# Tcadart/pyLatticeDSO

Measured on AMD Instinct MI355X. Metric: beams/s assembly+PCG-solve, higher is better.
Workload: dtype f64

## Files before the change

pylatticedso_amd/csrc/pl_api.hip:

```cpp
#include "pl_solver.h"
#include "pl_condense.h"
#include "pl_multi.h"


namespace {
template <typename WT>
int debug_spd_solve_t(int device, int32_t n, const double *A, const double *b, double *x, double *quad) {
  if (n <= 0 || !A || !b || !x) return fail(PL_ERR_ARG, "pl_debug_spd_solve: bad argument");
  int ndev = 0;
  if (hipGetDeviceCount(&ndev) != hipSuccess || ndev <= 0) return fail(PL_ERR_NODEVICE, "no HIP device visible");
  PL_HIP(hipSetDevice(device));
  const int np = (n + pl::kNB - 1) / pl::kNB * pl::kNB;
  std::vector<double> Ap((size_t)np * np, 0.0), bp(np, 0.0);
  for (int i = 0; i < np; ++i) {
    if (i < n) {
      std::memcpy(&Ap[(size_t)i * np], A + (size_t)i * n, n * sizeof(double));
      bp[i] = b[i];
    } else {
      Ap[(size_t)i * np + i] = 1.0;
    }
  }
  DevBuf<double> dA, dL, dD, db, dt, dy, dq;
  DevBuf<WT> dW, dWt;
  DevBuf<int> dinfo;
// ... 18 lines not shown
  PL_HIP(hipGetLastError());
  PL_HIP(hipDeviceSynchronize());
  int info[2];
  PL_HIP(hipMemcpy(info, dinfo.p, sizeof(info), hipMemcpyDeviceToHost));
  if (info[0] != 0) return fail(PL_ERR_ARG, "pl_debug_spd_solve: matrix is not positive definite");
  std::vector<double> y(np), q(pl::kSlots);
  PL_HIP(hipMemcpy(y.data(), dy.p, np * sizeof(double), hipMemcpyDeviceToHost));
  PL_HIP(hipMemcpy(q.data(), dq.p, pl::kSlots * sizeof(double), hipMemcpyDeviceToHost));
  std::memcpy(x, y.data(), n * sizeof(double));
  if (quad) {
    *quad = 0.0;
    for (double v : q) *quad += v;
  }
  return PL_OK;
}

}

extern "C" {

const char *pl_last_error(void) { return g_err.c_str(); }
#ifndef PL_KP_HASH
#define PL_KP_HASH "unknown"
#endif
const char *pl_version(void) { return "pylattice_hip 0.2 (gfx950) kp=" PL_KP_HASH; }

uint32_t pl_opts_size(void) { return (uint32_t)sizeof(pl_opts_t); }
uint32_t pl_stats_size(void) { return (uint32_t)sizeof(pl_stats_t); }
uint32_t pl_abi_version(void) { return PL_ABI_VERSION; }

int pl_default_opts(pl_opts_t *o, uint32_t struct_size) {
  if (!o) return fail(PL_ERR_ARG, "pl_default_opts: null argument");
  if (struct_size != sizeof(pl_opts_t))
    return fail(PL_ERR_ARG, "pl_default_opts: the caller's pl_opts_t has " + std::to_string(struct_size) +
                                " bytes, this library's " + std::to_string(sizeof(pl_opts_t)) +
                                " (ABI version " + std::to_string(PL_ABI_VERSION) + "): rebuild the binding against include/pylattice_hip.h");
  std::memset(o, 0, sizeof(*o));
  o->struct_size = (uint32_t)sizeof(pl_opts_t);
  o->abi_version = PL_ABI_VERSION;
  o->young = 1013.0;
  o->poisson = 0.3;
  o->kappa = 0.9;
  o->pen_coef = 1.5;
  o->device = 0;
  o->spmv_kernel = 0;
  o->precond = 1;
  o->reorder = 1;
  o->check_every = 0;
  return PL_OK;
}

namespace {
int check_opts_abi(const pl_opts_t *o, const char *who) {
  if (o->struct_size != sizeof(pl_opts_t) || o->abi_version != PL_ABI_VERSION)
    return fail(PL_ERR_ARG, std::string(who) + ": pl_opts_t was not initialised by pl_default_opts of this library (struct_size " +
                                std::to_string(o->struct_size) + " / abi " + std::to_string(o->abi_version) + ", expected " +
                                std::to_string(sizeof(pl_opts_t)) + " / " + std::to_string(PL_ABI_VERSION) + ")");
  return PL_OK;
}
inline bool multi_rank_handle(const pl_opts_t *o) { return o->grid_nodes > 0; }
inline int coarse_modes_of(const pl_opts_t *o, int64_t N = -1) {
  const bool tile12 = o->precond == 3 && o->tile_modes != 6;
  if (!tile12 || o->coarse_modes == 6) return 6;
  if (multi_rank_handle(o)) N = o->grid_nodes;
  return (o->coarse_modes == 12 || N < 0 || N >= 250000) ? 12 : 6;
}
inline int coarse_budget(const pl_opts_t *o, int64_t N) {
  const bool multi_rank = o->grid_nodes > 0;
  if (o->coarse_max_dofs > 0) return o->coarse_max_dofs;
  if (multi_rank) return (coarse_modes_of(o, N) == 12 && o->grid_nodes >= 2000000) ? 6144 : 3072;
  if (coarse_modes_of(o, N) == 12) return N >= 2000000 ? 6144 : (N >= 1000000 ? 3072 : (N >= 250000 ? 1536 : 768));
  return N >= 1000000 ? 3072 : 2100;
}
}

int pl_create(const pl_mesh_t *m, const pl_opts_t *o, pl_handle *out) {
  if (!m || !o || !out) return fail(PL_ERR_ARG, "pl_create: null argument");
  if (int rc_abi = check_opts_abi(o, "pl_create")) return rc_abi;
  StageTimer stage("pl_create");
  if (m->n_nodes <= 0 || m->n_beams <= 0) return fail(PL_ERR_ARG, "pl_create: empty mesh");
  if (m->n_nodes >= (1LL << 31) - 64 || m->n_beams >= (1LL << 31) - 64)
    return fail(PL_ERR_ARG, "pl_create: more than 2^31 nodes/struts per handle");
  if (!m->node_xyz || !m->beam_conn || !m->beam_radius || !m->seg_len || !m->seg_nsub)
    return fail(PL_ERR_ARG, "pl_create: null mesh array");
  int ndev = 0;
  if (hipGetDeviceCount(&ndev) != hipSuccess || ndev <= 0)
    return fail(PL_ERR_NODEVICE, "pl_create: no HIP device visible (libpylattice_hip has no CPU fallback)");
  if (o->device < 0 || o->device >= ndev) return fail(PL_ERR_ARG, "pl_create: bad device ordinal");
  if (o->precond == 5 && 6 * m->n_nodes > PL_DDM_DENSE_MAX)
    return fail(PL_ERR_ARG, "pl_create: precond = 5 (dense factorisation) serves at most PL_DDM_DENSE_MAX dofs");
  const int64_t N = m->n_nodes, B = m->n_beams;
  {
    std::atomic<int64_t> bad_ends{-1}, bad_radius{-1}, bad_len{-1}, bad_seg{-1};
    pl::parallel_for(B, [&](int64_t b0, int64_t b1, unsigned) {
      for (int64_t b = b0; b < b1; ++b) {
        const int32_t a = m->beam_conn[2 * b], d = m->beam_conn[2 * b + 1];
        if (a < 0 || d < 0 || a >= N || d >= N || a == d) bad_ends = b;
        if (!(m->beam_radius[b] > 0.0)) bad_radius = b;
        const double L = m->seg_len[3 * b] + m->seg_len[3 * b + 1] + m->seg_len[3 * b + 2];
        if (!(L > 0.0)) bad_len = b;
        for (int k = 0; k < 3; ++k)
          if (m->seg_len[3 * b + k] < 0.0 || (m->seg_len[3 * b + k] > 0.0 && m->seg_nsub[3 * b + k] < 1)) bad_seg = b;
      }
    });
    if (bad_ends >= 0)
      return fail(PL_ERR_ARG, "pl_create: strut " + std::to_string(bad_ends.load()) + " has invalid end nodes");
    if (bad_radius >= 0) return fail(PL_ERR_ARG, "pl_create: non-positive radius");
    if (bad_len >= 0) return fail(PL_ERR_ARG, "pl_create: strut with zero length");
    if (bad_seg >= 0) return fail(PL_ERR_ARG, "pl_create: bad segment data on strut " + std::to_string(bad_seg.load()));
  }
  stage.mark("validate");
  PL_HIP(hipSetDevice(o->device));
  pl_context *c = new pl_context();
  c->opt = *o;
  c->N = N;
  c->B = B;
  c->mat = {o->young, o->young / (2.0 * (1.0 + o->poisson)), o->kappa, o->pen_coef};
  c->lpn = o->lanes_per_node > 0 ? o->lanes_per_node : pl::kDefaultLPN;
  if (c->lpn != 1 && c->lpn != 2 && c->lpn != 4 && c->lpn != 8 && c->lpn != 16) {
    delete c;
    return fail(PL_ERR_ARG, "pl_create: lanes_per_node must be 0 (default), 1, 2, 4, 8 or 16");
  }
  auto bail = [&](int rc) {
    delete c;
    return rc;
  };
#define PL_TRY(expr)              \
  do {                            \
    int _rc = (expr);             \
    if (_rc) return bail(_rc);    \
  } while (0)
#define PL_HIPC(expr)                                                                  \
  do {                                                                                 \
    hipError_t _e = (expr);                                                            \
    if (_e != hipSuccess)                                                              \
      return bail(fail(PL_ERR_HIP, std::string(#expr) + ": " + hipGetErrorString(_e))); \
  } while (0)
  {
    int prio_low = 0, prio_high = 0;
    PL_HIPC(hipDeviceGetStreamPriorityRange(&prio_low, &prio_high));
    PL_HIPC(hipStreamCreateWithPriority(&c->stream, hipStreamNonBlocking, prio_high));
    PL_HIPC(hipStreamCreateWithPriority(&c->side, hipStreamNonBlocking, prio_low));
  }
  PL_HIPC(hipEventCreate(&c->ev0));
  PL_HIPC(hipEventCreate(&c->ev1));
  PL_HIPC(hipEventCreateWithFlags(&c->ev_fork, hipEventDisableTiming));
  PL_HIPC(hipEventCreateWithFlags(&c->ev_join, hipEventDisableTiming));
  PL_HIPC(hipEventCreateWithFlags(&c->ev_chol, hipEventDisableTiming));
  PL_HIPC(hipEventCreateWithFlags(&c->ev_t0, hipEventDisableTiming));
  PL_HIPC(hipEventCreateWithFlags(&c->ev_t1, hipEventDisableTiming));
  PL_HIPC(hipEventCreateWithFlags(&c->ev_p0, hipEventDisableTiming));
  PL_HIPC(hipEventCreateWithFlags(&c->ev_p1, hipEventDisableTiming));
  PL_HIPC(hipEventCreateWithFlags(&c->ev_fill1, hipEventDisableTiming));
  PL_HIPC(hipStreamCreateWithFlags(&c->side2, hipStreamNonBlocking));
  {
    const char *e = std::getenv("PL_BSR_CUMASK");
    const int k = e ? std::atoi(e) : 4;
    hipDeviceProp_t prop;
    const bool tuned_layout = hipGetDeviceProperties(&prop, o->device) == hipSuccess && prop.multiProcessorCount == 256;
    if (k > 0 && k < 8 && tuned_layout) {
      uint32_t mask[8];
      for (int w = 0; w < 8; ++w) {
        mask[w] = 0u;
        for (int b = 0; b < 32; ++b) {
          const int i = 32 * w + b;
          if ((i / 8 + i) % 8 >= k) mask[w] |= 1u << b;
        }
      }
      if (hipExtStreamCreateWithCUMask(&c->side_cu, 8, mask) != hipSuccess) {
        (void)hipGetLastError();
        c->side_cu = nullptr;
      }
    }
  }

  const double global_grid[7] = {o->grid_lo[0], o->grid_lo[1], o->grid_lo[2], o->grid_hi[0], o->grid_hi[1],
                                 o->grid_hi[2], (double)o->grid_nodes};
  c->perm.resize(N);
  std::iota(c->perm.begin(), c->perm.end(), 0);
  std::vector<int32_t> tile_start, tile_of;
  std::vector<int64_t> tile_brick;
  pl::BrickGrid grid;
  if (o->reorder == 1) {
    pl::spatial_order(m->node_xyz, N, c->perm, tile_start,
                      (double)(o->tile_nodes > 0 ? std::min(o->tile_nodes, pl::kTileMaxNodes) : 256), tile_brick,
                      grid, o->grid_nodes > 0 ? global_grid : nullptr,
                      (o->precond >= 2 && o->precond <= 4) ? coarse_budget(o, N) * 6 / coarse_modes_of(o, N) : 0);
    c->reordered = true;
    {
      std::vector<uint64_t> kind((size_t)N, 0);
      pl::parallel_for(B, [&](int64_t b0, int64_t b1, unsigned) {
        for (int64_t b = b0; b < b1; ++b) {
          const int32_t u = m->beam_conn[2 * b], v = m->beam_conn[2 * b + 1];
          uint64_t d = 0;
          for (int k = 0; k < 3; ++k) {
            const int64_t q = (int64_t)std::llround((m->node_xyz[3 * (size_t)v + k] - m->node_xyz[3 * (size_t)u + k]) * 4096.0);
            d = d * 0x9E3779B97F4A7C15ull + (uint64_t)(q + (1 << 20));
          }
          auto mix = [](uint64_t h) { h ^= h >> 33; h *= 0xFF51AFD7ED558CCDull; h ^= h >> 33; return h; };
          __atomic_fetch_add(&kind[u], mix(d), __ATOMIC_RELAXED);
          __atomic_fetch_add(&kind[v], mix(~d), __ATOMIC_RELAXED);
        }
      }, 1 << 16);
      const int64_t T = (int64_t)tile_start.size() - 1;
      pl::parallel_for(T, [&](int64_t t0, int64_t t1, unsigned) {
        for (int64_t t = t0; t < t1; ++t)
          std::stable_sort(c->perm.begin() + tile_start[t], c->perm.begin() + tile_start[t + 1],
                           [&](int32_t l, int32_t r) { return kind[l] < kind[r]; });
      }, 16);
    }
  } else {
    pl::chunk_tiles(N, tile_start);
  }
  stage.mark("spatial order");
  c->iperm.resize(N);
  pl::parallel_for(N, [&](int64_t i0, int64_t i1, unsigned) {
    for (int64_t i = i0; i < i1; ++i) c->iperm[c->perm[i]] = (int32_t)i;
  }, 1 << 16);
  if (o->condense >= 0 && o->precond >= 2 && o->precond <= 4 && o->precision != 2 && o->reorder == 1) {
    std::vector<int64_t> aptr((size_t)N + 1, 0);
    pl::parallel_for(2 * B, [&](int64_t k0, int64_t k1, unsigned) {
      for (int64_t k = k0; k < k1; ++k)
        __atomic_fetch_add(&aptr[c->iperm[m->beam_conn[k]] + 1], (int64_t)1, __ATOMIC_RELAXED);
    }, 1 << 16);
    for (int64_t i = 0; i < N; ++i) aptr[i + 1] += aptr[i];
    std::vector<int32_t> adj((size_t)2 * B);
    {
      std::vector<int64_t> fill(aptr.begin(), aptr.end() - 1);
      pl::parallel_for(B, [&](int64_t b0, int64_t b1, unsigned) {
        for (int64_t b = b0; b < b1; ++b) {
          const int32_t u = c->iperm[m->beam_conn[2 * b]], v = c->iperm[m->beam_conn[2 * b + 1]];
          adj[__atomic_fetch_add(&fill[u], (int64_t)1, __ATOMIC_RELAXED)] = v;
          adj[__atomic_fetch_add(&fill[v], (int64_t)1, __ATOMIC_RELAXED)] = u;
        }
      }, 1 << 16);
    }
    double lo[3] = {1e300, 1e300, 1e300}, hi[3] = {-1e300, -1e300, -1e300};
    for (int64_t i = 0; i < N; ++i)
      for (int k = 0; k < 3; ++k) {
        lo[k] = std::min(lo[k], m->node_xyz[3 * i + k]);
        hi[k] = std::max(hi[k], m->node_xyz[3 * i + k]);
      }
    std::vector<uint8_t> state((size_t)N, 0);
    for (int pass = 0; pass < 2; ++pass)
      for (int64_t i = 0; i < N; ++i) {
        if (state[i] || aptr[i + 1] - aptr[i] < 3) continue;
        const double *q3 = m->node_xyz + 3 * (size_t)c->perm[i];
        const bool on_box = q3[0] <= lo[0] || q3[0] >= hi[0] || q3[1] <= lo[1] || q3[1] >= hi[1] || q3[2] <= lo[2] ||
                            q3[2] >= hi[2];
        if (on_box != (pass == 1)) continue;
        state[i] = 1;
        for (int64_t q = aptr[i]; q < aptr[i + 1]; ++q)
          if (!state[adj[q]]) state[adj[q]] = 2;
      }
    int64_t n_cand = 0;
    for (int64_t i = 0; i < N; ++i) n_cand += state[i] == 1;
    const bool use = o->condense > 0 || (double)n_cand >= 0.45 * (double)N;
    const int64_t T = use ? (int64_t)tile_start.size() - 1 : 0;
    std::vector<int32_t> np(c->perm.size());
    if (use) c->h_cand.assign((size_t)N, 0);
    for (int64_t t = 0; t < T; ++t) {
      int64_t w = tile_start[t];
      for (int pass = 0; pass < 2; ++pass)
        for (int64_t i = tile_start[t]; i < tile_start[t + 1]; ++i)
          if ((state[i] == 1) == (pass == 1)) {
            c->h_cand[w] = (uint8_t)pass;
            np[w++] = c->perm[i];
          }
    }
    if (use) {
      c->perm.swap(np);
      for (int64_t i = 0; i < N; ++i) c->iperm[c->perm[i]] = (int32_t)i;
    }
  }

  stage.mark("candidates");
  std::vector<double> xyz((size_t)N * 3);
  pl::parallel_for(N, [&](int64_t i0, int64_t i1, unsigned) {
    for (int64_t i = i0; i < i1; ++i)
      std::memcpy(&xyz[3 * i], m->node_xyz + 3 * (size_t)c->perm[i], 3 * sizeof(double));
  });
  std::vector<int32_t> conn((size_t)B * 2);
  {
    std::vector<int32_t> conn0((size_t)B * 2);
    pl::parallel_for(2 * B, [&](int64_t k0, int64_t k1, unsigned) {
      for (int64_t k = k0; k < k1; ++k) conn0[k] = c->iperm[m->beam_conn[k]];
    });
    pl::tile_strut_order(conn0, N, B, tile_start, tile_of, c->bperm, xyz.data());
    pl::parallel_for(B, [&](int64_t b0, int64_t b1, unsigned) {
      for (int64_t b = b0; b < b1; ++b) {
        conn[2 * b] = conn0[2 * (size_t)c->bperm[b]];
        conn[2 * b + 1] = conn0[2 * (size_t)c->bperm[b] + 1];
      }
    });
  }
  stage.mark("strut order");
  std::vector<double> radius(B), seg_len((size_t)B * 3);
  std::vector<int32_t> seg_nsub((size_t)B * 3);
  pl::parallel_for(B, [&](int64_t b0, int64_t b1, unsigned) {
    for (int64_t b = b0; b < b1; ++b) {
      const size_t ob = (size_t)c->bperm[b];
      radius[b] = m->beam_radius[ob];
      for (int k = 0; k < 3; ++k) {
        seg_len[3 * b + k] = m->seg_len[3 * ob + k];
        seg_nsub[3 * b + k] = m->seg_nsub[3 * ob + k];
      }
    }
// ... 400 lines not shown
    if (cell_S[c] < 0 || cell_S[c] >= n_S) return fail(PL_ERR_ARG, "pl_ddm_set_preconditioner: matrix id out of range");
  const int m = 6 * h->ddm_nb;
  std::vector<double> Pt((size_t)n_S * m * m);
  for (int s = 0; s < n_S; ++s)
    for (int i = 0; i < m; ++i)
      for (int j = 0; j < m; ++j) Pt[((size_t)s * m + j) * m + i] = S[((size_t)s * m + i) * m + j];
  PL_HIP(h->ddm_Pt.alloc(Pt.size()));
  PL_HIP(h->ddm_cell_P.alloc(h->ddm_cells));
  PL_HIP(hipMemcpy(h->ddm_Pt.p, Pt.data(), Pt.size() * sizeof(double), hipMemcpyHostToDevice));
  PL_HIP(hipMemcpy(h->ddm_cell_P.p, cell_S, h->ddm_cells * sizeof(int32_t), hipMemcpyHostToDevice));
  h->ddm_have_P = true;
  return PL_OK;
}

static int ensure_bsr_buffers(pl_context *h) {
  if (h->bsr_vals.p) return PL_OK;
  PL_HIP(h->bsr_rowptr.alloc(h->N + 1));
  PL_HIP(h->bsr_col.alloc(h->nblk));
  PL_HIP(h->bsr_vals.alloc((size_t)h->nblk * 36));
  PL_HIP(hipMemcpy(h->bsr_rowptr.p, h->h_rowptr.data(), (h->N + 1) * sizeof(int64_t), hipMemcpyHostToDevice));
  PL_HIP(hipMemcpy(h->bsr_col.p, h->h_col.data(), h->nblk * sizeof(int32_t), hipMemcpyHostToDevice));
  return PL_OK;
}

static int ddm_factor_preconditioner(pl_context *h) {
  const int64_t n6 = h->N * 6;
  const int np = (int)((n6 + pl::kNB - 1) / pl::kNB * pl::kNB);
  if (h->dd_n != np) {
    const size_t nn = (size_t)np * np;
    PL_HIP(h->dd_A.alloc(nn));
    PL_HIP(h->dd_Lf.alloc(nn));
    PL_HIP(h->dd_W.alloc(nn));
    PL_HIP(h->dd_Wt.alloc(nn));
    PL_HIP(h->dd_Dinv.alloc((size_t)np * pl::kNB));
    PL_HIP(h->dd_tv.alloc(np));
    PL_HIP(h->dd_info.alloc(2));
    PL_HIP(hipMemsetAsync(h->dd_W.p, 0, nn * sizeof(double), h->stream));
    PL_HIP(hipMemsetAsync(h->dd_Wt.p, 0, nn * sizeof(double), h->stream));
    h->dd_n = np;
  }
  h->dd_ready = false;
  PL_HIP(hipMemsetAsync(h->dd_A.p, 0, (size_t)np * np * sizeof(double), h->stream));
  PL_HIP(hipMemsetAsync(h->dd_info.p, 0, 2 * sizeof(int), h->stream));
  const int m = 6 * h->ddm_nb;
  const int64_t ne = h->ddm_cells * m * m;
  const uint8_t *fx = h->have_bc ? h->fixed.p : (const uint8_t *)nullptr;
  hipLaunchKernelGGL(pl::k_ddm_dense_assemble, dim3(grid_for(ne)), dim3(pl::kBlock), 0, h->stream, h->ddm_cells,
                     h->ddm_nb, h->ddm_cell_nodes.p, h->ddm_have_P ? h->ddm_cell_P.p : h->ddm_cell_S.p,
                     h->ddm_have_P ? h->ddm_Pt.p : h->ddm_St.p, fx, np, h->dd_A.p);
  hipLaunchKernelGGL(pl::k_ddm_dense_unit, dim3((np + 255) / 256), dim3(256), 0, h->stream, n6, np, fx, h->dd_A.p);
  pl::dense_factor_inverse(h->dd_A.p, h->dd_Lf.p, h->dd_W.p, h->dd_Wt.p, h->dd_Dinv.p, np, np, h->dd_info.p,
                           h->dd_bw, h->stream);
  PL_HIP(hipGetLastError());
  int info[2] = {0, 0};
  PL_HIP(hipMemcpyAsync(info, h->dd_info.p, sizeof(info), hipMemcpyDeviceToHost, h->stream));
  PL_HIP(hipStreamSynchronize(h->stream));
  h->dd_ready = (info[0] == 0);
  return PL_OK;
}

static int fem_factor_dense(pl_context *h) {
  const int64_t n6 = h->N * 6;
  const int np = (int)((n6 + pl::kNB - 1) / pl::kNB * pl::kNB);
  if (h->dd_n != np) {
    const size_t nn = (size_t)np * np;
    PL_HIP(h->dd_A.alloc(nn));
    PL_HIP(h->dd_Lf.alloc(nn));
    PL_HIP(h->dd_W.alloc(nn));
    PL_HIP(h->dd_Wt.alloc(nn));
    PL_HIP(h->dd_Dinv.alloc((size_t)np * pl::kNB));
    PL_HIP(h->dd_tv.alloc(np));
    PL_HIP(h->dd_info.alloc(2));
    PL_HIP(hipMemsetAsync(h->dd_W.p, 0, nn * sizeof(double), h->stream));
    PL_HIP(hipMemsetAsync(h->dd_Wt.p, 0, nn * sizeof(double), h->stream));
    h->dd_n = np;
    int64_t band = 0;
    for (int64_t i = 0; i < h->N; ++i)
      for (int64_t q = h->h_rowptr[i]; q < h->h_rowptr[i + 1]; ++q) band = std::max<int64_t>(band, std::llabs((long long)(h->h_col[q] - i)));
    h->dd_bw = (int)((6 * (band + 1) + pl::kNB - 1) / pl::kNB + 1);
  }
  h->dd_ready = false;
  int rc = ensure_bsr_buffers(h);
  if (rc) return rc;
  PL_HIP(hipMemsetAsync(h->dd_A.p, 0, (size_t)np * np * sizeof(double), h->stream));
  PL_HIP(hipMemsetAsync(h->dd_info.p, 0, 2 * sizeof(int), h->stream));
  rc = launch_bsr_fill(h, 1, h->stream);
  if (rc) return rc;
  h->have_bsr = false;
  hipLaunchKernelGGL(pl::k_bsr_to_dense, dim3(grid_for(h->nblk * 36)), dim3(pl::kBlock), 0, h->stream, h->N, h->nblk,
                     h->bsr_rowptr.p, h->bsr_col.p, (const double *)h->bsr_vals.p, np, h->dd_A.p);
  hipLaunchKernelGGL(pl::k_ddm_dense_unit, dim3((np + 255) / 256), dim3(256), 0, h->stream, n6, np, (const uint8_t *)nullptr,
                     h->dd_A.p);
  pl::dense_factor_inverse(h->dd_A.p, h->dd_Lf.p, h->dd_W.p, h->dd_Wt.p, h->dd_Dinv.p, np, np, h->dd_info.p, h->dd_bw,
                           h->stream);
  PL_HIP(hipGetLastError());
  int info[2] = {0, 0};
  PL_HIP(hipMemcpyAsync(info, h->dd_info.p, sizeof(info), hipMemcpyDeviceToHost, h->stream));
  PL_HIP(hipStreamSynchronize(h->stream));
  h->dd_ready = (info[0] == 0);
  if (h->dd_ready) PL_HIP(hipMemsetAsync(h->dinv.p, 0, n6 * sizeof(double), h->stream));
  return PL_OK;
}

void pl_destroy(pl_handle h) {
  if (!h) return;
  (void)hipSetDevice(h->opt.device);
  (void)hipStreamSynchronize(h->stream);
  if (h->comm_stream) (void)hipStreamSynchronize(h->comm_stream);
  pl::dist_destroy(h->dist);
  if (h->pal_host_flags != h->pal_fallback_flags) (void)hipHostFree(h->pal_host_flags);
  if (h->cls_host_flag) (void)hipHostFree(h->cls_host_flag);
  delete h;
}

int pl_set_bc(pl_handle h, const uint8_t *fixed, const double *ubar, const double *f) {
  if (!valid(h) || !fixed) return fail(PL_ERR_ARG, "pl_set_bc: null argument");
  PL_HIP(hipSetDevice(h->opt.device));
  const int64_t N = h->N;
  const size_t n6 = (size_t)N * 6;
  std::vector<uint8_t> fx(n6), bits(N);
  double *st = nullptr;
  if (int rcs = staging(h, &st)) return rcs;
  pl::parallel_for(N, [&](int64_t i0, int64_t i1, unsigned) {
    for (int64_t i = i0; i < i1; ++i) {
      const size_t src = 6 * (size_t)h->perm[i];
      uint8_t b = 0;
      for (int k = 0; k < 6; ++k) {
        const uint8_t v = fixed[src + k] ? 1 : 0;
        fx[6 * i + k] = v;
        b |= (uint8_t)(v << k);
        st[6 * i + k] = (ubar && v) ? ubar[src + k] : 0.0;
      }
      bits[i] = b;
    }
  }, 1 << 15);
  PL_HIP(hipMemcpyAsync(h->ubar.p, st, n6 * sizeof(double), hipMemcpyHostToDevice, h->stream));
  PL_HIP(hipMemcpyAsync(h->fixed.p, fx.data(), n6, hipMemcpyHostToDevice, h->stream));
  PL_HIP(hipMemcpyAsync(h->fixedbits.p, bits.data(), N, hipMemcpyHostToDevice, h->stream));
  PL_HIP(hipStreamSynchronize(h->stream));
  pl::parallel_for(N, [&](int64_t i0, int64_t i1, unsigned) {
    for (int64_t i = i0; i < i1; ++i) {
      const size_t src = 6 * (size_t)h->perm[i];
      for (int k = 0; k < 6; ++k) st[6 * i + k] = f ? f[src + k] : 0.0;
    }
  }, 1 << 15);
  PL_HIP(hipMemcpyAsync(h->f.p, st, n6 * sizeof(double), hipMemcpyHostToDevice, h->stream));
  PL_HIP(hipStreamSynchronize(h->stream));
  const bool same_mask = h->have_bc && !h->dist.active && h->h_fixedbits == bits;
  h->h_fixedbits = bits;
  if (same_mask) return PL_OK;
  h->have_bc = true;
  h->coarse.n_fix = -1;
  h->coarseL.n_fix = -1;
  {
    int rcs = select_condensed(h, bits);
    if (rcs) return rcs;
  }
  if (h->assembled && h->opkind == 1) {
    if (h->opt.precond >= 2 && h->opt.precond <= 4) {
      h->assembled = false;
      h->dd_ready = false;
      h->dd_blocks = false;
      h->dd2_ready = false;
    } else {
      pl::launch_invert_diag(h->N * 6, h->diag.p, h->fixed.p, h->dinv.p, h->stream);
      PL_HIP(hipStreamSynchronize(h->stream));
    }
  } else if (h->assembled) {
    int rc = launch_diag(h, h->stream);
    if (rc) return rc;
    rc = finish_diag_dist(h);
    if (rc) return rc;
    rc = launch_local_mask(h);
    if (rc) return rc;
    rc = launch_tile_blocks(h, h->stream);
    if (rc) return rc;
    rc = build_coarse(h);
    if (rc) return rc;
    rc = launch_dinv32(h);
    if (rc) return rc;
    rc = agree_condensed(h);
    if (rc) return rc;
    rc = launch_condensed_blocks(h, h->stream);
    if (rc) return rc;
    PL_HIP(hipStreamSynchronize(h->stream));
    {
      const bool keep = h->pal_ready;
      finish_condensed_classes(h);
      (void)keep;
    }
    if (h->bsr_with_bc) h->have_bsr = false;
    if (h->opt.precond == 5 && !h->dist.active) {
      rc = fem_factor_dense(h);
      if (rc) return rc;
    }
  }
  return PL_OK;
}

int pl_set_periodic(pl_handle h, const int32_t *master) {
  if (!valid(h)) return fail(PL_ERR_ARG, "pl_set_periodic: null handle");
  if (h->opkind != 0) return fail(PL_ERR_STATE, "pl_set_periodic: not available on a DDM handle");
  h->n_per_groups = 0;
  if (!master) return PL_OK;
  if (h->opt.precond != 1 || h->dist.active)
    return fail(PL_ERR_STATE, "pl_set_periodic: periodic constraints are served by the Jacobi PCG of a single-GPU handle (opts.precond = 1)");
  PL_HIP(hipSetDevice(h->opt.device));
  const int64_t N = h->N;
  std::vector<int32_t> inv((size_t)N);
  for (int64_t i = 0; i < N; ++i) inv[(size_t)h->perm[i]] = (int32_t)i;
  std::vector<int32_t> cnt((size_t)N, 0);
  for (int64_t i = 0; i < N; ++i) {
    const int32_t m = master[i];
    if (m < 0 || m >= N || master[m] != m) return fail(PL_ERR_ARG, "pl_set_periodic: master[i] must name a node that is its own master");
    cnt[(size_t)m]++;
  }
  std::vector<int32_t> ptr(1, 0), nodes, start((size_t)N, -1);
  for (int64_t m = 0; m < N; ++m)
    if (cnt[(size_t)m] >= 2) {
      start[(size_t)m] = (int32_t)ptr.size() - 1;
      ptr.push_back(ptr.back() + cnt[(size_t)m]);
    }
  nodes.resize((size_t)ptr.back());
  std::vector<int32_t> fill(ptr.begin(), ptr.end() - 1);
  for (int64_t i = 0; i < N; ++i) {
    const int32_t g = start[(size_t)master[i]];
    if (g >= 0) nodes[(size_t)fill[(size_t)g]++] = inv[(size_t)i];
  }
  const int64_t ng = (int64_t)ptr.size() - 1;
  if (ng == 0) return PL_OK;
  PL_HIP(h->per_ptr.alloc(ptr.size()));
  PL_HIP(h->per_nodes.alloc(nodes.size()));
  PL_HIP(hipMemcpy(h->per_ptr.p, ptr.data(), ptr.size() * sizeof(int32_t), hipMemcpyHostToDevice));
  PL_HIP(hipMemcpy(h->per_nodes.p, nodes.data(), nodes.size() * sizeof(int32_t), hipMemcpyHostToDevice));
  h->n_per_groups = ng;
  return PL_OK;
}

int pl_update_radii(pl_handle h, const double *beam_radius) {
  if (!valid(h) || !beam_radius) return fail(PL_ERR_ARG, "pl_update_radii: null argument");
  if (h->opkind != 0) return fail(PL_ERR_STATE, "pl_update_radii: not available on a DDM handle");
  for (int64_t b = 0; b < h->B; ++b)
    if (!(beam_radius[b] > 0.0)) return fail(PL_ERR_ARG, "pl_update_radii: non-positive radius");
  PL_HIP(hipSetDevice(h->opt.device));
  double *stg = nullptr;
  int rc = stagingB(h, &stg);
  if (rc) return rc;
  pl::parallel_for(h->B, [&](int64_t b0, int64_t b1, unsigned) {
    for (int64_t b = b0; b < b1; ++b) stg[b] = beam_radius[h->bperm[b]];
  }, 1 << 16);
  PL_HIP(hipMemcpyAsync(h->radius.p, stg, h->B * sizeof(double), hipMemcpyHostToDevice, h->stream));
  PL_HIP(hipStreamSynchronize(h->stream));
  h->assembled = false;
  h->have_bsr = false;
  return PL_OK;
}

int pl_set_multiplicity(pl_handle h, const double *beam_mult) {
  if (!valid(h)) return fail(PL_ERR_ARG, "pl_set_multiplicity: null handle");
  if (h->opkind != 0) return fail(PL_ERR_STATE, "pl_set_multiplicity: not available on a DDM handle");
  PL_HIP(hipSetDevice(h->opt.device));
  if (!beam_mult) {
    h->mult.release();
  } else {
    for (int64_t b = 0; b < h->B; ++b)
      if (!(beam_mult[b] > 0.0)) return fail(PL_ERR_ARG, "pl_set_multiplicity: non-positive multiplicity");
    std::vector<double> m(h->B);
    for (int64_t b = 0; b < h->B; ++b) m[b] = beam_mult[h->bperm[b]];
    if (!h->mult.p) PL_HIP(h->mult.alloc(h->B));
    PL_HIP(hipMemcpy(h->mult.p, m.data(), h->B * sizeof(double), hipMemcpyHostToDevice));
  }
  h->assembled = false;
  h->have_bsr = false;
  return PL_OK;
}

int pl_update_segments(pl_handle h, const double *seg_len, const int32_t *seg_nsub) {
  if (!valid(h) || !seg_len || !seg_nsub) return fail(PL_ERR_ARG, "pl_update_segments: null argument");
  PL_HIP(hipSetDevice(h->opt.device));
  std::vector<double> sl((size_t)h->B * 3);
  std::vector<int32_t> sn((size_t)h->B * 3);
  for (int64_t b = 0; b < h->B; ++b)
    for (int k = 0; k < 3; ++k) {
      sl[3 * b + k] = seg_len[3 * (size_t)h->bperm[b] + k];
      sn[3 * b + k] = seg_nsub[3 * (size_t)h->bperm[b] + k];
    }
  PL_HIP(hipMemcpy(h->seg_len.p, sl.data(), 3 * h->B * sizeof(double), hipMemcpyHostToDevice));
  PL_HIP(hipMemcpy(h->seg_nsub.p, sn.data(), 3 * h->B * sizeof(int32_t), hipMemcpyHostToDevice));
  h->assembled = false;
  h->have_bsr = false;
  return PL_OK;
}

int pl_assemble(pl_handle h) {
  if (!valid(h)) return fail(PL_ERR_ARG, "pl_assemble: null handle");
  PL_HIP(hipSetDevice(h->opt.device));
  if (h->opkind == 1) {
    if (h->assembled && (h->opt.precond == 0 || (h->opt.precond == 1 && !h->dd_ready && !h->dd_blocks) || h->dd_ready || h->dd_blocks)) {
      h->ms_assembly = 0.0;
      return PL_OK;
    }
    h->dd_ready = false;
    h->dd_blocks = false;
    h->dd2_ready = false;
    if (h->opt.precond == 4 && !h->dd2_plan)
      return fail(PL_ERR_STATE, "pl_assemble: precond = 4 on a DDM handle needs the node positions (pl_ddm_set_geometry)");
    if (h->opt.precond == 3 || h->opt.precond == 4) {
      PL_HIP(hipEventRecord(h->ev0, h->stream));
      if (!h->dd_B.p) PL_HIP(h->dd_B.alloc((size_t)h->N * 36));
      PL_HIP(hipMemsetAsync(h->dd_B.p, 0, (size_t)h->N * 36 * sizeof(double), h->stream));
      const int64_t ne = (int64_t)h->ddm_cells * h->ddm_nb * 36;
      hipLaunchKernelGGL(pl::k_ddm_node_blocks, dim3(grid_for(ne)), dim3(pl::kBlock), 0, h->stream, h->ddm_cells, h->ddm_nb,
                         h->ddm_cell_nodes.p, h->ddm_have_P ? h->ddm_cell_P.p : h->ddm_cell_S.p,
                         h->ddm_have_P ? h->ddm_Pt.p : h->ddm_St.p, h->dd_B.p);
      hipLaunchKernelGGL(pl::k_ddm_node_blocks_invert, dim3(grid_for(h->N)), dim3(pl::kBlock), 0, h->stream, h->N,
                         h->have_bc ? (const uint8_t *)h->fixed.p : (const uint8_t *)nullptr, h->dd_B.p);
      PL_HIP(hipMemsetAsync(h->dinv.p, 0, h->N * 6 * sizeof(double), h->stream));
      int info2[2] = {0, 0};
      if (h->opt.precond == 4) {
        pl::Coarse &cs = h->dd2;
        const int n = cs.ncp, m = 6 * h->ddm_nb;
        PL_HIP(hipMemsetAsync(cs.Ac, 0, (size_t)n * n * sizeof(double), h->stream));
        PL_HIP(hipMemsetAsync(cs.info, 0, 2 * sizeof(int), h->stream));
        hipLaunchKernelGGL(pl::k_ddm_coarse_cells, dim3((unsigned)h->ddm_cells), dim3(pl::kWave),
                           (size_t)2 * m * pl::kDdmModes * sizeof(double), h->stream, h->ddm_cells, h->ddm_nb,
                           h->ddm_cell_nodes.p, h->ddm_have_P ? h->ddm_cell_P.p : h->ddm_cell_S.p,
                           h->ddm_have_P ? h->ddm_Pt.p : h->ddm_St.p, h->dd2_agg.p, h->dd2_cen.p, h->dd2_xyz.p,
                           h->have_bc ? (const uint8_t *)h->fixed.p : (const uint8_t *)nullptr, n, cs.Ac);
        hipLaunchKernelGGL(pl::k_coarse_regularize, dim3((n + 255) / 256), dim3(256), 0, h->stream, n, cs.Ac);
        pl::TrtriPhases ph;
        ph.rows = 3;
        ph.stream = h->side2;
        ph.ev_go = h->ev_t0;
        ph.ev_done = h->ev_t1;
        pl::coarse_factor(cs, n, h->stream, nullptr, (unsigned *)nullptr, ph);
        cs.ainv_ready = false;
        if (cs.Ainv) {
          const long tiles = (long)(n / 32) * (n / 32 + 1) / 2;
          if (cs.w16)
            hipLaunchKernelGGL(pl::k_dense_explicit_inverse<pl::bf16_t>, dim3((unsigned)((tiles + 3) / 4)), dim3(256), 0,
                               h->stream, n, reinterpret_cast<const pl::bf16_t *>(cs.W), n, cs.Ainv);
          else
            hipLaunchKernelGGL(pl::k_dense_explicit_inverse<float>, dim3((unsigned)((tiles + 3) / 4)), dim3(256), 0, h->stream,
                               n, (const float *)cs.W, n, cs.Ainv);
          cs.ainv_ready = true;
        }
        PL_HIP(hipMemcpyAsync(info2, cs.info, sizeof(info2), hipMemcpyDeviceToHost, h->stream));
      }
      PL_HIP(hipEventRecord(h->ev1, h->stream));
      PL_HIP(hipEventSynchronize(h->ev1));
      PL_HIP(hipGetLastError());
      float ms = 0.f;
      PL_HIP(hipEventElapsedTime(&ms, h->ev0, h->ev1));
      h->ms_assembly = ms;
      h->dd2_ready = h->opt.precond == 4 && info2[0] == 0;
      h->dd_blocks = true;
      h->assembled = true;
      return PL_OK;
    }
    if (h->opt.precond == 2) {
      PL_HIP(hipEventRecord(h->ev0, h->stream));
      int rcp = ddm_factor_preconditioner(h);
      if (rcp) return rcp;
      if (h->dd_ready) {
        PL_HIP(hipMemsetAsync(h->dinv.p, 0, h->N * 6 * sizeof(double), h->stream));
        PL_HIP(hipEventRecord(h->ev1, h->stream));
        PL_HIP(hipEventSynchronize(h->ev1));
        float ms = 0.f;
        PL_HIP(hipEventElapsedTime(&ms, h->ev0, h->ev1));
        h->ms_assembly = ms;
        h->assembled = true;
        return PL_OK;
      }
    }
    if (h->opt.precond >= 1) {
      PL_HIP(hipMemsetAsync(h->diag.p, 0, h->N * 6 * sizeof(double), h->stream));
      const int64_t m = (int64_t)h->ddm_cells * h->ddm_nb * 6;
      hipLaunchKernelGGL(pl::k_ddm_diag, dim3(grid_for(m)), dim3(pl::kBlock), 0, h->stream, h->ddm_cells, h->ddm_nb,
                         h->ddm_cell_nodes.p, h->ddm_cell_S.p, h->ddm_St.p, h->diag.p);
    } else {
      pl::launch_fill(h->N * 6, 1.0, h->diag.p, h->stream);
    }
    pl::launch_invert_diag(h->N * 6, h->diag.p, h->have_bc ? h->fixed.p : nullptr, h->dinv.p, h->stream);
    PL_HIP(hipStreamSynchronize(h->stream));
    h->ms_assembly = 0.0;
    h->assembled = true;
    return PL_OK;
  }
  int rc = agree_condensed(h);
  if (rc) return rc;
  PL_HIP(hipEventRecord(h->ev0, h->stream));
  rc = launch_records(h);
  if (rc) return rc;
  rc = launch_local_mask(h);
  if (rc) return rc;
  PL_HIP(hipEventRecord(h->ev_fork, h->stream));
  PL_HIP(hipStreamWaitEvent(h->side, h->ev_fork, 0));
  rc = launch_palette(h, h->side);
  if (rc) return rc;
  rc = launch_diag(h, h->dist.active ? h->stream : h->side);
  if (rc) return rc;
  rc = finish_diag_dist(h);
  if (rc) return rc;
  rc = launch_tile_blocks(h, h->side);
  if (rc) return rc;
  rc = launch_condensed_blocks(h, h->side);
  if (rc) return rc;
  const bool refresh_bsr = h->want_bsr && (!h->bsr_with_bc || h->have_bc);
  int rc_fill = PL_OK;
  bool fill_queued = false;
  int64_t split = 0;
  if (refresh_bsr && h->side_cu && h->coarse.enabled && h->have_bc) {
    static const double kChainLinkMs = [] { const char *e = std::getenv("PL_CHAIN_LINK_MS"); return e ? std::atof(e) : 0.04; }();
    static const double kFillBlocksPerMs = [] { const char *e = std::getenv("PL_FILL_BLOCKS_PER_MS"); return e ? std::atof(e) : 8.5e6; }();
    const double chain_ms = kChainLinkMs * std::max(0, h->coarse.ncp / pl::kNB - 1);
    const double fit = chain_ms * kFillBlocksPerMs / std::max<double>(1.0, (double)h->nblk);
    split = fit >= 1.0 ? h->n_slices : (int64_t)(fit * (double)h->n_slices);
    if (split < h->n_slices / 16) split = 0;
  }
  bool part1_queued = false;
  auto queue_fill = [&](int phase) {
    if (!refresh_bsr || fill_queued) return;
    if (phase == 0) {
      if (split <= 0 || part1_queued) return;
      part1_queued = true;
      if (hipEventRecord(h->ev_chol, h->stream) != hipSuccess || hipStreamWaitEvent(h->side_cu, h->ev_chol, 0) != hipSuccess ||
          hipStreamWaitEvent(h->side_cu, h->ev_join, 0) != hipSuccess) {
        rc_fill = fail(PL_ERR_HIP, "pl_assemble: could not order the BSR fill beside the factorisation");
        return;
      }
      rc_fill = launch_bsr_fill(h, h->bsr_with_bc, h->side_cu, 0, split);
      if (hipEventRecord(h->ev_fill1, h->side_cu) != hipSuccess) rc_fill = fail(PL_ERR_HIP, "pl_assemble: event record failed");
      return;
    }
    fill_queued = true;
    if (hipEventRecord(h->ev_chol, h->stream) != hipSuccess || hipStreamWaitEvent(h->side, h->ev_chol, 0) != hipSuccess) {
      rc_fill = fail(PL_ERR_HIP, "pl_assemble: could not order the BSR fill behind the factorisation");
      return;
    }
    if (!rc_fill) rc_fill = launch_bsr_fill(h, h->bsr_with_bc, h->side, part1_queued ? split : 0, -1);
    if (part1_queued && hipStreamWaitEvent(h->side, h->ev_fill1, 0) != hipSuccess)
      rc_fill = fail(PL_ERR_HIP, "pl_assemble: event wait failed");
    if (hipEventRecord(h->ev_join, h->side) != hipSuccess) rc_fill = fail(PL_ERR_HIP, "pl_assemble: event record failed");
  };
  PL_HIP(hipEventRecord(h->ev_join, h->side));
  h->dd_ready = false;
  if (h->opt.precond == 5 && h->have_bc && !h->dist.active) {
    PL_HIP(hipStreamWaitEvent(h->stream, h->ev_join, 0));
    rc = fem_factor_dense(h);
    if (rc) return rc;
  }
  rc = build_coarse(h, h->coarse.enabled && h->have_bc ? std::function<void(int)>(queue_fill) : std::function<void(int)>());
  if (rc) return rc;
  queue_fill(1);
  if (rc_fill) return rc_fill;
  PL_HIP(hipStreamWaitEvent(h->stream, h->ev_join, 0));
  rc = launch_dinv32(h);
  if (rc) return rc;
  PL_HIP(hipEventRecord(h->ev1, h->stream));
  PL_HIP(hipStreamSynchronize(h->stream));
  finish_palette(h);
  finish_condensed_classes(h);
  for (pl::Coarse *cs : {&h->coarse, &h->coarseL})
    if (cs->ready && cs->Ac) {
      PL_HIP(hipMemsetAsync(cs->Ac, 0, (size_t)cs->ncp * cs->ncp * sizeof(double), h->stream));
      cs->ac_clean = true;
    }
  float ms = 0.f;
  PL_HIP(hipEventElapsedTime(&ms, h->ev0, h->ev1));
  h->ms_assembly = ms;
  h->assembled = true;
  h->have_bsr = refresh_bsr;
  return PL_OK;
}

int pl_assemble_bsr(pl_handle h, int with_bc, int64_t *n_block_rows, int64_t *n_blocks) {
  if (!valid(h)) return fail(PL_ERR_ARG, "pl_assemble_bsr: null handle");
  if (h->opkind != 0) return fail(PL_ERR_STATE, "pl_assemble_bsr: not available on a DDM handle");
  if (!h->assembled) return fail(PL_ERR_STATE, "pl_assemble_bsr: call pl_assemble first");
  if (with_bc && !h->have_bc) return fail(PL_ERR_STATE, "pl_assemble_bsr: with_bc needs pl_set_bc");
  PL_HIP(hipSetDevice(h->opt.device));
  if (int rcb = ensure_bsr_buffers(h)) return rcb;
  const bool fresh = h->have_bsr && h->want_bsr && h->bsr_with_bc == (with_bc ? 1 : 0);
  h->want_bsr = true;
  h->bsr_with_bc = with_bc ? 1 : 0;
  if (fresh) {
    if (n_block_rows) *n_block_rows = h->N;
    if (n_blocks) *n_blocks = h->nblk;
    return PL_OK;
  }
  PL_HIP(hipEventRecord(h->ev0, h->stream));
  int rc = launch_bsr_fill(h, with_bc, h->stream);
  if (rc) return rc;
  PL_HIP(hipEventRecord(h->ev1, h->stream));
  PL_HIP(hipStreamSynchronize(h->stream));
  float ms = 0.f;
  PL_HIP(hipEventElapsedTime(&ms, h->ev0, h->ev1));
  h->ms_assembly += ms;
  h->have_bsr = true;
  if (n_block_rows) *n_block_rows = h->N;
  if (n_blocks) *n_blocks = h->nblk;
  return PL_OK;
}

int pl_get_bsr(pl_handle h, int64_t *rowptr, int32_t *colidx, double *vals) {
  if (!valid(h)) return fail(PL_ERR_ARG, "pl_get_bsr: null handle");
  if (!h->have_bsr) return fail(PL_ERR_STATE, "pl_get_bsr: call pl_assemble_bsr first");
  PL_HIP(hipSetDevice(h->opt.device));
  std::vector<double> v((size_t)h->nblk * 36);
  PL_HIP(hipMemcpy(v.data(), h->bsr_vals.p, v.size() * sizeof(double), hipMemcpyDeviceToHost));
  if (!h->reordered) {
    if (rowptr) std::memcpy(rowptr, h->h_rowptr.data(), (h->N + 1) * sizeof(int64_t));
    if (colidx) std::memcpy(colidx, h->h_col.data(), h->nblk * sizeof(int32_t));
    if (vals) std::memcpy(vals, v.data(), v.size() * sizeof(double));
    return PL_OK;
  }
  std::vector<int64_t> rp(h->N + 1, 0);
  for (int64_t ci = 0; ci < h->N; ++ci) {
    const int64_t di = h->iperm[ci];
    rp[ci + 1] = rp[ci] + (h->h_rowptr[di + 1] - h->h_rowptr[di]);
  }
  if (rowptr) std::memcpy(rowptr, rp.data(), (h->N + 1) * sizeof(int64_t));
  std::vector<std::pair<int32_t, int64_t>> row;
  for (int64_t ci = 0; ci < h->N; ++ci) {
    const int64_t di = h->iperm[ci];
    row.clear();
    for (int64_t p = h->h_rowptr[di]; p < h->h_rowptr[di + 1]; ++p) row.push_back({h->perm[h->h_col[p]], p});
    std::stable_sort(row.begin(), row.end(), [](auto &l, auto &r) { return l.first < r.first; });
    for (size_t k = 0; k < row.size(); ++k) {
      if (colidx) colidx[rp[ci] + k] = row[k].first;
      if (vals) std::memcpy(vals + 36 * (rp[ci] + k), &v[36 * row[k].second], 36 * sizeof(double));
    }
  }
  return PL_OK;
}

static int spmv_common(pl_handle h, const double *x, double *y, bool masked, const char *who) {
  if (!valid(h) || !x || !y) return fail(PL_ERR_ARG, std::string(who) + ": null argument");
  if (!h->assembled) return fail(PL_ERR_STATE, std::string(who) + ": call pl_assemble first");
  if (masked && !h->have_bc) return fail(PL_ERR_STATE, std::string(who) + ": call pl_set_bc first");
  PL_HIP(hipSetDevice(h->opt.device));
  std::vector<double> stage;
  int rc = upload6(h, x, h->tmp.p, stage);
  if (rc) return rc;
  if (masked) {
    hipLaunchKernelGGL(pl::k_mask_dot, dim3(grid_stream(h->N * 6)), dim3(pl::kBlock), 0, h->stream, h->N * 6,
                       h->fixed.p, h->tmp.p, h->tmp.p, (double *)nullptr);
  }
  rc = launch_spmv(h, h->tmp.p, h->tmp2.p, masked, nullptr);
  if (rc) return rc;
  return download6(h, h->tmp2.p, y);
}

int pl_spmv(pl_handle h, const double *x, double *y) { return spmv_common(h, x, y, false, "pl_spmv"); }
int pl_spmv_free(pl_handle h, const double *x, double *y) { return spmv_common(h, x, y, true, "pl_spmv_free"); }

int pl_spmv_bsr(pl_handle h, const double *x, double *y) {
  if (!valid(h) || !x || !y) return fail(PL_ERR_ARG, "pl_spmv_bsr: null argument");
  if (!h->have_bsr) return fail(PL_ERR_STATE, "pl_spmv_bsr: call pl_assemble_bsr first");
  PL_HIP(hipSetDevice(h->opt.device));
  std::vector<double> stage;
  int rc = upload6(h, x, h->tmp.p, stage);
  if (rc) return rc;
  hipLaunchKernelGGL(pl::k_bsr_spmv, dim3(grid_for(h->N)), dim3(pl::kBlock), 0, h->stream, h->N, h->bsr_rowptr.p,
                     h->bsr_col.p, h->bsr_vals.p, h->tmp.p, h->tmp2.p);
  PL_HIP(hipGetLastError());
  return download6(h, h->tmp2.p, y);
}

int pl_solve(pl_handle h, double rtol, int32_t max_iter, double *u, pl_stats_t *stats) {
  if (!valid(h)) return fail(PL_ERR_ARG, "pl_solve: null handle");
  if (!h->assembled) return fail(PL_ERR_STATE, "pl_solve: call pl_assemble first");
  if (!h->have_bc) return fail(PL_ERR_STATE, "pl_solve: call pl_set_bc first");
  if (!(rtol > 0.0) || max_iter <= 0) return fail(PL_ERR_ARG, "pl_solve: rtol and max_iter must be positive");
  if (stats && stats->struct_size != sizeof(pl_stats_t))
    return fail(PL_ERR_ARG, "pl_solve: stats->struct_size is " + std::to_string(stats->struct_size) + ", this library's pl_stats_t has " +
                                std::to_string(sizeof(pl_stats_t)) + " bytes (set it to sizeof(pl_stats_t) before the call)");
  PL_HIP(hipSetDevice(h->opt.device));
  const int64_t n6 = h->N * 6;
  pl_stats_t st{};
  st.struct_size = (uint32_t)sizeof(pl_stats_t);
  PL_HIP(hipEventRecord(h->ev0, h->stream));
  int rc = launch_spmv(h, h->ubar.p, h->tmp.p, false, nullptr);
  if (rc) return rc;
  if (h->n_per_groups > 0 && (h->coarse.ready || ref_cg(h) || h->dist.active))
    return fail(PL_ERR_STATE, "pl_solve: periodic constraints (pl_set_periodic) need the plain Jacobi PCG");
  const bool mp = mp_applies(h);
  solver_plan(h);
  const bool cg1 = !mp && cg1_applies(h);
  st.cg_form_used = cg1 ? 1.0 : 0.0;
  if (cg1) rc = pcg_solve_cg1(h, h->f.p, h->tmp.p, rtol, max_iter, &st);
  else if (mp && h->opt.precision == 1) rc = pcg_solve_mp_t<float>(h, h->f.p, h->tmp.p, rtol, max_iter, &st);
  else if (mp) rc = pcg_solve_mp_t<double>(h, h->f.p, h->tmp.p, rtol, max_iter, &st);
  else rc = pcg_solve(h, h->f.p, h->tmp.p, rtol, max_iter, &st);
  if (rc) return rc;
  st.precision_used = mp ? (double)h->opt.precision : 0.0;
  st.kp_form = (double)kp_form_of(h);
  st.comm_world = h->dist.active ? (double)h->dist.comm_count : 0.0;
  st.comm_rank = h->dist.active ? (double)h->dist.comm_user_rank : 0.0;
  st.condensed_nodes = h->cond_use ? (double)h->n_cond : 0.0;
  if (st.converged) st.info = 0.0;
  else if (st.info != 2.0) st.info = 1.0;
  if (!h->usol.p) PL_HIP(h->usol.alloc((size_t)n6));
  h->usol_valid = false;
  hipLaunchKernelGGL(pl::k_compose_solution, dim3(grid_stream(n6)), dim3(pl::kBlock), 0, h->stream, n6, h->fixed.p,
                     h->ubar.p, h->x.p, h->usol.p);
  PL_HIP(hipEventRecord(h->ev1, h->stream));
  PL_HIP(hipStreamSynchronize(h->stream));
  float ms = 0.f;
  PL_HIP(hipEventElapsedTime(&ms, h->ev0, h->ev1));
  st.ms_solve = ms;
  st.ms_assembly = h->ms_assembly;
  st.precond_used = h->opkind == 1 ? (h->dd_ready ? 2 : h->dd2_ready ? 4 : h->dd_blocks ? 3 : h->opt.precond >= 1 ? 1 : 0)
                                   : (h->coarse.ready ? h->opt.precond : (h->dd_ready ? 5 : 1));
// ... 452 lines not shown
  a.nb = nb;
  a.ni = ni;
  a.conn = dconn.p;
  a.end_slot = dslot.p;
  a.node_slot = dnslot.p;
  a.xyz = dxyz.p;
  a.radius = drad.p;
  a.seg_len = dlen.p;
  a.seg_nsub = dnsub.p;
  a.m = {o->young, o->young / (2.0 * (1.0 + o->poisson)), o->kappa, o->pen_coef};
  a.u_b = dub.p;
  a.lam_b = lam_b ? dlb.p : nullptr;
  a.u_full = u_full ? duf.p : nullptr;
  a.lam_full = lam_full ? dlf.p : nullptr;
  a.sens = sens ? dsens.p : nullptr;
  a.info = dinfo.p;
  if (lds > 64 * 1024)
    PL_HIP(hipFuncSetAttribute(reinterpret_cast<const void *>(&pl::k_cells_recover),
                               hipFuncAttributeMaxDynamicSharedMemorySize, (int)lds));
  KernelEventTimer kernel_time("pl_cells_recover", stage.on);
  hipLaunchKernelGGL(pl::k_cells_recover, dim3((unsigned)n_inst), dim3((unsigned)block), lds, nullptr, a);
  kernel_time.stop();
  PL_HIP(hipGetLastError());
  PL_HIP(hipDeviceSynchronize());
  kernel_time.report();
  stage.mark("kernel");
  if (u_full) PL_HIP(hipMemcpy(u_full, duf.p, duf.n * sizeof(double), hipMemcpyDeviceToHost));
  if (lam_full) PL_HIP(hipMemcpy(lam_full, dlf.p, dlf.n * sizeof(double), hipMemcpyDeviceToHost));
  if (sens) PL_HIP(hipMemcpy(sens, dsens.p, dsens.n * sizeof(double), hipMemcpyDeviceToHost));
  PL_HIP(hipMemcpy(info, dinfo.p, ninst * sizeof(int32_t), hipMemcpyDeviceToHost));
  stage.mark("download");
  return PL_OK;
}

int pl_get_records(pl_handle h, double *rec) {
  if (!valid(h) || !rec) return fail(PL_ERR_ARG, "pl_get_records: null argument");
  if (!h->assembled) return fail(PL_ERR_STATE, "pl_get_records: call pl_assemble first");
  PL_HIP(hipSetDevice(h->opt.device));
  std::vector<pl::Record> tmp(h->B);
  PL_HIP(hipMemcpy(tmp.data(), h->rec.p, h->B * sizeof(pl::Record), hipMemcpyDeviceToHost));
  for (int64_t b = 0; b < h->B; ++b) std::memcpy(rec + 8 * (size_t)h->bperm[b], &tmp[b], sizeof(pl::Record));
  return PL_OK;
}

int pl_algorithmic_bytes(pl_handle h, double *out3) {
  if (!valid(h) || !out3) return fail(PL_ERR_ARG, "pl_algorithmic_bytes: null argument");
  const double w = 8.0, B = (double)h->B, N = (double)h->N;
  const bool mp = h->assembled && mp_applies(h);
  const double wv = mp ? 4.0 : 8.0;
  const double wx = (mp && h->opt.precision == 1) ? 4.0 : 8.0;
  out3[0] = B * (8.0 + 8.0 * w) + N * 6.0 * wv * 2.0;
  out3[1] = out3[0] + 10.0 * (6.0 * N * wx);
  out3[2] = B * (8.0 + 8.0 * w) + (N + 2.0 * B) * (36.0 * w + 4.0);
  return PL_OK;
}

int pl_forget_history(pl_handle h) {
  if (!valid(h)) return fail(PL_ERR_ARG, "pl_forget_history: null handle");
  h->last_iterations = 0;
  h->xprev_valid = false;
  h->xprev2_valid = false;
  h->xprev3_valid = false;
  h->gh_count = 0;
  return PL_OK;
}

int pl_time_kernel(pl_handle h, int which, int reps, double *avg_ms) {
  if (!valid(h) || !avg_ms || reps <= 0) return fail(PL_ERR_ARG, "pl_time_kernel: bad argument");
  if (h->opkind != 0 && which != 0 && which != 3 && which != 10 && which != 11) return fail(PL_ERR_STATE, "pl_time_kernel: DDM handles time K*p / PCG only");
  if (!h->assembled) return fail(PL_ERR_STATE, "pl_time_kernel: call pl_assemble first");
  if ((which == 0 || which == 3 || which == 10 || which == 11) && !h->have_bc) return fail(PL_ERR_STATE, "pl_time_kernel: call pl_set_bc first");
  if ((which == 2 || which == 4) && !h->have_bsr) return fail(PL_ERR_STATE, "pl_time_kernel: needs pl_assemble_bsr");
  PL_HIP(hipSetDevice(h->opt.device));
  const int64_t n6 = h->N * 6;
  int rc = ensure_hist(h, reps + 1);
  if (rc) return rc;
  solver_plan(h);
  h->stop_use = false;
  if (h->small_use && (which == 3 || which == 11)) {
    rc = small_prepare(h);
    if (rc) return rc;
  }
  PL_HIP(hipMemcpyAsync(h->p.p, h->dinv.p, n6 * sizeof(double), hipMemcpyDeviceToDevice, h->stream));
  if (which >= 7 && which <= 11) {
    hipLaunchKernelGGL(pl::k_to_float, dim3(grid_for(n6)), dim3(pl::kBlock), 0, h->stream, n6, h->dinv.p,
                       reinterpret_cast<float *>(h->z.p));
    PL_HIP(hipMemsetAsync(h->tmp.p, 0, n6 * sizeof(double), h->stream));
  }
  auto one = [&](int k) -> int {
    switch (which) {
      case 0: return launch_spmv(h, h->p.p, h->Ap.p, true, h->scal.p + pl::S_PAP * pl::kSlots);
      case 1: {
        int r1 = launch_records(h);
        return r1 ? r1 : build_palette(h);
      }
      case 2: return launch_bsr_fill(h, 0, h->stream);
      case 3: return pcg_iteration(h, k);
      case 4:
        hipLaunchKernelGGL(pl::k_bsr_spmv, dim3(grid_for(h->N)), dim3(pl::kBlock), 0, h->stream, h->N,
                           h->bsr_rowptr.p, h->bsr_col.p, h->bsr_vals.p, h->p.p, h->Ap.p);
        return PL_OK;
      case 5:
        if (!h->dist.active) return fail(PL_ERR_STATE, "pl_time_kernel: 5/6 need pl_dist_init");
        return pl::dist_sum_shared(h->dist, h->Ap.p, h->stream, h->scal.p + pl::S_PAP * pl::kSlots, pl::kSlots)
                   ? fail(PL_ERR_HIP, "RCCL all-reduce failed") : PL_OK;
      case 6:
        if (!h->dist.active || !h->coarse.ready) return fail(PL_ERR_STATE, "pl_time_kernel: 6 needs a coarse level");
        return pl::dist_sum_scalars(h->dist, h->coarse.tv, h->coarse.ncp, h->stream)
                   ? fail(PL_ERR_HIP, "RCCL all-reduce failed") : PL_OK;
      case 7:
      case 8:
      case 9: {
        if (!(h->coarse.ready && h->tile.ready && choose_kernel(h) == 3))
          return fail(PL_ERR_STATE, "pl_time_kernel: 7/8/9 need the multi-level PCG on the tile kernel");
        float *p32 = reinterpret_cast<float *>(h->z.p), *Ap32 = p32 + n6;
        double *cur = h->scal.p + (k & 1) * pl::S_COUNT * pl::kSlots, *nxt = h->scal.p + ((k + 1) & 1) * pl::S_COUNT * pl::kSlots;
        int r7 = launch_spmv_f32(h, p32, Ap32, true, cur + pl::S_PAP * pl::kSlots);
        if (r7 || which == 7) return r7;
        if (which == 8) {
          float *x32 = reinterpret_cast<float *>(h->tmp.p), *r32 = x32 + n6;
          return pcg_tail_coarse_t<float, float>(h, cur, nxt, k, p32, (const float *)Ap32, x32, r32);
        }
        return pcg_tail_coarse_t<float, double>(h, cur, nxt, k, p32, (const float *)Ap32, h->x.p, h->r.p);
      }
      case 10: {
        if (mp_applies(h)) {
          float *p32 = reinterpret_cast<float *>(h->z.p), *Ap32 = p32 + n6;
          if (h->cond_use) {
            int r0 = launch_spmv_f32(h, p32, p32, false, nullptr, nullptr, pl::kEndsCondensedSolve);
            return r0 ? r0 : launch_spmv_f32(h, p32, Ap32, true, h->scal.p + pl::S_PAP * pl::kSlots, h->maskC.p, pl::kEndsOthers);
          }
          return launch_spmv_f32(h, p32, Ap32, true, h->scal.p + pl::S_PAP * pl::kSlots);
        }
        if (h->cond_use) {
          int r0 = launch_spmv(h, h->p.p, h->p.p, false, nullptr, nullptr, pl::kEndsCondensedSolve);
          return r0 ? r0 : launch_spmv(h, h->p.p, h->Ap.p, true, h->scal.p + pl::S_PAP * pl::kSlots, h->maskC.p, pl::kEndsOthers);
        }
        return launch_spmv(h, h->p.p, h->Ap.p, true, h->scal.p + pl::S_PAP * pl::kSlots);
      }
      case 11: {
        if (!(mp_applies(h) && h->opt.precision == 1)) return pcg_iteration(h, k);
        float *p32 = reinterpret_cast<float *>(h->z.p), *Ap32 = p32 + n6;
        float *x32 = reinterpret_cast<float *>(h->tmp.p), *r32 = x32 + n6;
        double *cur = h->scal.p + (k & 1) * pl::S_COUNT * pl::kSlots, *nxt = h->scal.p + ((k + 1) & 1) * pl::S_COUNT * pl::kSlots;
        int r11;
        if (h->cond_use) {
          r11 = launch_spmv_f32(h, p32, p32, false, nullptr, nullptr, pl::kEndsCondensedSolve);
          if (!r11) r11 = launch_spmv_f32(h, p32, Ap32, true, cur + pl::S_PAP * pl::kSlots, h->maskC.p, pl::kEndsOthers);
        } else {
          r11 = launch_spmv_f32(h, p32, Ap32, true, cur + pl::S_PAP * pl::kSlots);
        }
        return r11 ? r11 : pcg_tail_coarse_t<float, float>(h, cur, nxt, k, p32, (const float *)Ap32, x32, r32);
      }
      default: return fail(PL_ERR_ARG, "pl_time_kernel: unknown kernel id");
    }
  };
  for (int k = 0; k < 3; ++k) {
    rc = one(0);
    if (rc) return rc;
  }
  PL_HIP(hipEventRecord(h->ev0, h->stream));
  for (int k = 0; k < reps; ++k) {
    rc = one(k);
    if (rc) return rc;
  }
  PL_HIP(hipEventRecord(h->ev1, h->stream));
  PL_HIP(hipStreamSynchronize(h->stream));
  float ms = 0.f;
  PL_HIP(hipEventElapsedTime(&ms, h->ev0, h->ev1));
  *avg_ms = (double)ms / reps;
  return PL_OK;
}

int pl_debug_spd_solve(int device, int32_t n, const double *A, const double *b, double *x, double *quad,
                       int32_t fp32_factor) {
  return fp32_factor ? debug_spd_solve_t<float>(device, n, A, b, x, quad)
                     : debug_spd_solve_t<double>(device, n, A, b, x, quad);
}

int pl_lzone(int device, int64_t n_nodes, int64_t n_beams, const double *node_xyz, const int32_t *beam_conn,
             const double *beam_radius, double *lzone) {
  if (n_nodes <= 0 || n_beams <= 0 || !node_xyz || !beam_conn || !beam_radius || !lzone)
    return fail(PL_ERR_ARG, "pl_lzone: bad argument");
  int ndev = 0;
  if (hipGetDeviceCount(&ndev) != hipSuccess || ndev <= 0)
    return fail(PL_ERR_NODEVICE, "pl_lzone: no HIP device visible (libpylattice_hip has no CPU fallback)");
  if (device < 0 || device >= ndev) return fail(PL_ERR_ARG, "pl_lzone: bad device ordinal");
  const int64_t nh = 2 * n_beams;
  std::vector<int64_t> ptr((size_t)n_nodes + 1, 0);
  for (int64_t h = 0; h < nh; ++h) {
    const int32_t v = beam_conn[h];
    if (v < 0 || v >= n_nodes) return fail(PL_ERR_ARG, "pl_lzone: node id out of range");
    ptr[(size_t)v + 1]++;
  }
  for (int64_t i = 0; i < n_nodes; ++i) ptr[i + 1] += ptr[i];
  std::vector<int32_t> half((size_t)nh);
  {
    std::vector<int64_t> fill(ptr.begin(), ptr.end() - 1);
    for (int64_t h = 0; h < nh; ++h) half[(size_t)fill[beam_conn[h]]++] = (int32_t)h;
  }
  PL_HIP(hipSetDevice(device));
  DevBuf<double> dx, dr, dl;
  DevBuf<int32_t> dc, dh;
  DevBuf<int64_t> dp;
  PL_HIP(dx.alloc((size_t)n_nodes * 3));
  PL_HIP(dr.alloc(n_beams));
  PL_HIP(dl.alloc(nh));
  PL_HIP(dc.alloc(nh));
  PL_HIP(dh.alloc(nh));
  PL_HIP(dp.alloc(n_nodes + 1));
  PL_HIP(hipMemcpy(dx.p, node_xyz, (size_t)n_nodes * 3 * sizeof(double), hipMemcpyHostToDevice));
  PL_HIP(hipMemcpy(dr.p, beam_radius, n_beams * sizeof(double), hipMemcpyHostToDevice));
  PL_HIP(hipMemcpy(dc.p, beam_conn, nh * sizeof(int32_t), hipMemcpyHostToDevice));
  PL_HIP(hipMemcpy(dh.p, half.data(), nh * sizeof(int32_t), hipMemcpyHostToDevice));
  PL_HIP(hipMemcpy(dp.p, ptr.data(), (n_nodes + 1) * sizeof(int64_t), hipMemcpyHostToDevice));
  hipLaunchKernelGGL(pl::k_lzone, dim3(grid_for(nh)), dim3(pl::kBlock), 0, nullptr, nh, dx.p, dc.p, dr.p, dp.p, dh.p,
                     dl.p);
  PL_HIP(hipGetLastError());
  PL_HIP(hipMemcpy(lzone, dl.p, nh * sizeof(double), hipMemcpyDeviceToHost));
  return PL_OK;
}

#ifdef PL_TILE_STAMPS
int pl_debug_tile_stamps(unsigned long long *out) {
  return hipMemcpyFromSymbol(out, HIP_SYMBOL(pl::g_tile_stamps), sizeof(unsigned long long) * 8 * 4096) == hipSuccess ? 0 : -2;
}
#endif

int pl_dist_unique_id_bytes(void) { return pl::dist_unique_id_bytes(); }
int pl_dist_unique_id(void *id_out) {
  if (!id_out) return fail(PL_ERR_ARG, "pl_dist_unique_id: null argument");
  return pl::dist_unique_id(id_out) ? fail(PL_ERR_HIP, "ncclGetUniqueId failed") : PL_OK;
}
int pl_dist_loopback_id(void *id_out) {
  if (!id_out) return fail(PL_ERR_ARG, "pl_dist_loopback_id: null argument");
  pl::dist_loopback_id(id_out);
  return PL_OK;
}
int pl_dist_init(pl_handle h, int rank, int world, const void *unique_id, const int32_t *shared_local,
                 const int32_t *shared_global, int32_t n_shared, int32_t n_shared_global) {
  if (!valid(h) || !unique_id || world < 1 || rank < 0 || rank >= world || n_shared < 0)
    return fail(PL_ERR_ARG, "pl_dist_init: bad argument");
  if (n_shared > 0 && (!shared_local || !shared_global)) return fail(PL_ERR_ARG, "pl_dist_init: null index array");
  PL_HIP(hipSetDevice(h->opt.device));
  std::vector<int32_t> loc(n_shared);
  for (int i = 0; i < n_shared; ++i) {
    if (shared_local[i] < 0 || shared_local[i] >= h->N || shared_global[i] < 0 || shared_global[i] >= n_shared_global)
      return fail(PL_ERR_ARG, "pl_dist_init: shared node index out of range");
    loc[i] = h->iperm[shared_local[i]];
  }
  int rc = pl::dist_init(h->dist, rank, world, unique_id, loc.data(), shared_global, n_shared, n_shared_global, h->N,
                         h->stream);
  if (rc == 6)
    return fail(PL_ERR_ARG, "pl_dist_init: loopback group mismatch (all ranks of a loopback id must share one device and one "
                            "world size <= " + std::to_string(pl::kLoopMaxWorld) + ", each rank attaches once)");
  if (rc) return fail(PL_ERR_HIP, "pl_dist_init: communicator setup failed (" + std::to_string(rc) + ")");
  h->h_shared.assign((size_t)h->N, 0);
  for (int i = 0; i < n_shared; ++i) h->h_shared[loc[i]] = 1;
  h->ov_ready = false;
  if (h->coarse.enabled) {
    h->cond_ready = false;
    h->n_cond = 0;
    h->cond_agree = -1;
    PL_HIP(hipMemcpy(h->sharedbits.p, h->h_shared.data(), h->h_shared.size(), hipMemcpyHostToDevice));
    h->coarseL.n_fix = -1;
  }
  h->assembled = false;
  return PL_OK;
}

int pl_dist_abort(pl_handle h) {
  if (!valid(h)) return fail(PL_ERR_ARG, "pl_dist_abort: null handle");
  if (h->dist.loop) {
    std::lock_guard<std::mutex> lk(h->dist.loop->m);
    h->dist.loop->broken = true;
    h->dist.loop->cv.notify_all();
  }
  return PL_OK;
}

int pl_dist_set_peers(pl_handle h, const int32_t *shared_peer) {
  if (!valid(h) || !shared_peer) return fail(PL_ERR_ARG, "pl_dist_set_peers: null argument");
  if (!h->dist.active) return fail(PL_ERR_STATE, "pl_dist_set_peers: call pl_dist_init first");
  PL_HIP(hipSetDevice(h->opt.device));
  int rc = pl::dist_set_peers(h->dist, shared_peer);
  if (rc) return fail(rc == 2 ? PL_ERR_ARG : PL_ERR_HIP, "pl_dist_set_peers: setup failed (" + std::to_string(rc) + ")");
  h->assembled = false;
  h->ov_ready = false;
  if (h->opt.overlap >= 0 && h->tile.ready && h->opkind == 0 && !h->h_tile_start.empty()) {
    const int64_t T = (int64_t)h->h_tile_start.size() - 1;
    std::vector<int32_t> iface, inner;
    for (int64_t t = 0; t < T; ++t) {
      bool has = false;
      for (int32_t i = h->h_tile_start[t]; i < h->h_tile_start[t + 1] && !has; ++i) has = h->h_shared[i] != 0;
      (has ? iface : inner).push_back((int32_t)t);
    }
    if (!iface.empty() && !inner.empty()) {
      PL_HIP(h->ov_iface.alloc(iface.size()));
      PL_HIP(h->ov_inner.alloc(inner.size()));
      PL_HIP(hipMemcpy(h->ov_iface.p, iface.data(), iface.size() * sizeof(int32_t), hipMemcpyHostToDevice));
      PL_HIP(hipMemcpy(h->ov_inner.p, inner.data(), inner.size() * sizeof(int32_t), hipMemcpyHostToDevice));
      h->n_ov_iface = (int64_t)iface.size();
      h->n_ov_inner = (int64_t)inner.size();
      if (!h->comm_stream) {
        int prio_low = 0, prio_high = 0;
        PL_HIP(hipDeviceGetStreamPriorityRange(&prio_low, &prio_high));
        PL_HIP(hipStreamCreateWithPriority(&h->comm_stream, hipStreamNonBlocking, prio_high));
        PL_HIP(hipEventCreateWithFlags(&h->ev_ov_a, hipEventDisableTiming));
        PL_HIP(hipEventCreateWithFlags(&h->ev_ov_x, hipEventDisableTiming));
      }
      h->ov_ready = true;
    }
  }
  return PL_OK;
}

}
```

pylatticedso_amd/csrc/pl_assembly.h:

```cpp
#pragma once
#include "pl_ops.h"

namespace {

inline bool small_wanted(const pl_context *c) {
  const pl::Coarse &cs = c->coarse;
  if (c->opt.short_iteration < 0 || c->opkind != 0 || c->dist.active || c->coarseL.enabled || c->opt.precision != 0 ||
      c->opt.cg_form == 1 || !cs.enabled || !c->tile.ready || choose_kernel(c) != 3 || c->opt.mintol > 0.0 ||
      c->opt.restart_every > 0)
    return false;
  if (c->opt.short_iteration == 1) return true;
  static const double auto_mb = [] { const char *e = std::getenv("PL_SHORT_ITERATION_MB"); return e ? std::atof(e) : 16.0; }();
  return (double)cs.n_tiles * cs.cm * cs.ncp * 4.0 <= auto_mb * 1048576.0;
}


int launch_records(pl_context *c) {
  hipLaunchKernelGGL(pl::k_build_records, dim3(grid_for(c->B)), dim3(pl::kBlock), 0, c->stream, c->B, c->xyz.p,
                     c->conn.p, c->radius.p, c->seg_len.p, c->seg_nsub.p, c->mult.p, c->mat, c->rec.p, c->rec5.p);
  PL_HIP(hipGetLastError());
  return PL_OK;
}

void refresh_visit_words(pl_context *c, hipStream_t st) {
  if (c->rword.p && c->pal_dense_of_slot.p)
    hipLaunchKernelGGL(pl::k_row_words, dim3(grid_for(c->rows.n_words)), dim3(pl::kBlock), 0, st, c->rows.n_words,
                       c->rows.rloc.p, c->rows.rstrut.p, c->pal_id.p, c->pal_dense_of_slot.p, c->rword.p);
  if (!c->vword.p || !c->pal_dense_of_slot.p) return;
  hipLaunchKernelGGL(pl::k_visit_words, dim3(grid_for(c->tile.n_visits)), dim3(pl::kBlock), 0, st, c->tile.n_visits,
                     c->tile.vloc.p, c->tile.vstrut.p, c->pal_id.p, c->pal_dense_of_slot.p,
                     c->cend.p ? (const uint8_t *)c->cend.p : (const uint8_t *)nullptr, c->vword.p);
}
int refresh_visit_words_dir(pl_context *c, hipStream_t st) {
  if (!c->tile.vis_ready || c->tile.n_dir <= 0 || !c->rec5.p) return PL_OK;
  if (!c->vword_dir.p) PL_HIP(c->vword_dir.alloc((size_t)c->tile.n_visits));
  hipLaunchKernelGGL(pl::k_visit_words, dim3(grid_for(c->tile.n_visits)), dim3(pl::kBlock), 0, st, c->tile.n_visits,
                     c->tile.vloc.p, c->tile.vstrut.p, (const uint16_t *)nullptr, (const int *)nullptr,
                     c->cend.p ? (const uint8_t *)c->cend.p : (const uint8_t *)nullptr, c->vword_dir.p);
  c->vword_dir_fresh = true;
  return PL_OK;
}

int launch_palette(pl_context *c, hipStream_t st) {
  c->pal_ready = false;
  c->pal_lds = false;
  c->pal_rows = false;
  c->pal_host_flags[0] = 1;
  c->pal_host_flags[1] = 0;
  if (!c->vword_dir_fresh) {
    int rcw = refresh_visit_words_dir(c, st);
    if (rcw) return rcw;
  }
  if (!c->opt.palette) return PL_OK;
  c->pal_skipped = false;
  if (c->pal_skip_left > 0) {
    c->pal_skip_left--;
    c->pal_skipped = true;
    return PL_OK;
  }
  if (!c->pal_keys.p) {
    PL_HIP(c->pal_keys.alloc(pl::kPalSize));
    PL_HIP(c->pal_owner.alloc(pl::kPalSize));
    PL_HIP(c->pal_flags.alloc(2));
    PL_HIP(c->pal_id.alloc(c->B));
    PL_HIP(c->palette.alloc(pl::kPalSize));
    PL_HIP(c->pal_dense_of_slot.alloc(pl::kPalSize));
    PL_HIP(c->pal_dense.alloc(pl::kPalDenseMax));
    if (c->tile.vis_ready) PL_HIP(c->vword.alloc((size_t)c->tile.n_visits));
    if (c->rows.ready) {
      PL_HIP(c->rword.alloc((size_t)c->rows.n_words));
      PL_HIP(c->pal_dense2.alloc((size_t)2 * pl::kPalDenseMax));
    }
    void *pinned = nullptr;
    PL_HIP(hipHostMalloc(&pinned, 2 * sizeof(int), hipHostMallocDefault));
    c->pal_host_flags = static_cast<int *>(pinned);
    c->pal_host_flags[0] = 1;
    c->pal_host_flags[1] = 0;
  }
  PL_HIP(hipMemsetAsync(c->pal_keys.p, 0xFF, pl::kPalSize * sizeof(unsigned long long), st));
  PL_HIP(hipMemsetAsync(c->pal_owner.p, 0x7F, pl::kPalSize * sizeof(int), st));
  PL_HIP(hipMemsetAsync(c->pal_flags.p, 0, 2 * sizeof(int), st));
  PL_HIP(hipMemsetAsync(c->palette.p, 0, pl::kPalSize * sizeof(pl::Record), st));
  const dim3 g(grid_for(c->B)), blk(pl::kBlock);
  hipLaunchKernelGGL(pl::k_pal_insert, g, blk, 0, st, c->B, c->rec.p, c->pal_keys.p, c->pal_owner.p, c->pal_id.p,
                     c->pal_flags.p);
  hipLaunchKernelGGL(pl::k_pal_publish, g, blk, 0, st, c->B, c->rec.p, c->pal_owner.p, c->pal_id.p, c->palette.p);
  hipLaunchKernelGGL(pl::k_pal_verify, g, blk, 0, st, c->B, c->rec.p, c->pal_id.p, c->palette.p, c->pal_owner.p,
                     c->pal_flags.p, c->pal_dense_of_slot.p, c->pal_dense.p, pl::kPalDenseMax);
  refresh_visit_words(c, st);
  if (c->pal_dense2.p)
    hipLaunchKernelGGL(pl::k_pal_orient, dim3(1), dim3(pl::kPalDenseMax), 0, st, pl::kPalDenseMax, c->pal_dense.p,
                       c->pal_dense2.p);
  PL_HIP(hipGetLastError());
  PL_HIP(hipMemcpyAsync(c->pal_host_flags, c->pal_flags.p, 2 * sizeof(int), hipMemcpyDeviceToHost, st));
  return PL_OK;
}
void finish_palette(pl_context *c) {
  if (!c->opt.palette) return;
  if (c->pal_skipped) {
    c->pal_entries = 0;
    c->pal_ready = false;
    c->pal_lds = false;
    c->pal_rows = false;
    return;
  }
  c->pal_entries = c->pal_host_flags[1];
  c->pal_ready = (c->pal_host_flags[0] == 0);
  static const bool lds_off = [] { const char *e = std::getenv("PL_TILE_LDS"); return e && e[0] == '0'; }();
  c->pal_lds = c->pal_ready && c->vword.p && c->pal_entries > 0 && c->pal_entries <= pl::kPalDenseMax && !lds_off;
  if (c->pal_ready && !c->pal_lds && !lds_off && small_wanted(c) && c->rec5.p && c->vword_dir.p && c->tile.n_dir > 0 &&
      c->tile.n_dir <= pl::kPalDenseMax)
    c->pal_ready = false;
  if (c->pal_ready) {
    c->pal_fail_streak = 0;
  } else {
    c->pal_fail_streak = std::min(c->pal_fail_streak + 1, 4);
    c->pal_skip_left = (1 << c->pal_fail_streak) - 1;
  }
  const char *re = std::getenv("PL_ROWS");
  c->pal_rows = c->pal_lds && c->rword.p && c->pal_dense2.p && re && re[0] == '1';
}
int build_palette(pl_context *c) {
  int rc = launch_palette(c, c->stream);
  if (rc) return rc;
  PL_HIP(hipStreamSynchronize(c->stream));
  finish_palette(c);
  return PL_OK;
}

int launch_diag(pl_context *c, hipStream_t st) {
  const unsigned g = grid_for(c->n_slices, pl::kBlock / pl::kWave);
  const uint8_t *fb = c->have_bc ? c->fixedbits.p : (const uint8_t *)nullptr;
#define PL_D(L)                                                                                                  \
  hipLaunchKernelGGL((pl::k_diag_gather<L>), dim3(g), dim3(pl::kBlock), 0, st, c->N, c->slice_ptr.p, c->ent.p, \
                     c->rec.p, fb, c->diag.p, c->dinv.p)
  switch (c->lpn) { case 1: PL_D(1); break; case 2: PL_D(2); break; case 4: PL_D(4); break; case 8: PL_D(8); break;
                    default: PL_D(16); }
#undef PL_D
  PL_HIP(hipGetLastError());
  return PL_OK;
}
int finish_diag_dist(pl_context *c) {
  if (!c->dist.active) return PL_OK;
  int rc = pl::dist_sum_shared(c->dist, c->diag.p, c->stream);
  if (rc) return fail(PL_ERR_HIP, "RCCL all-reduce of the Jacobi diagonal failed");
  pl::launch_invert_diag(c->N * 6, c->diag.p, c->have_bc ? c->fixed.p : nullptr, c->dinv.p, c->stream);
  return PL_OK;
}

__global__ void k_local_mask(int64_t N, const uint8_t *__restrict__ fixedbits, const uint8_t *__restrict__ shared,
                             uint8_t *__restrict__ mask) {
  const int64_t i = (int64_t)blockIdx.x * blockDim.x + threadIdx.x;
  if (i < N) mask[i] = (uint8_t)(fixedbits[i] | (shared[i] ? 0x3f : 0));
}

int launch_dinv32(pl_context *c) {
  if (!c->coarse.enabled) return PL_OK;
  hipLaunchKernelGGL(pl::k_to_float, dim3(grid_for(c->N * 6)), dim3(pl::kBlock), 0, c->stream, c->N * 6, c->dinv.p,
                     c->coarse.dinv32);
  PL_HIP(hipGetLastError());
  return PL_OK;
}

int launch_local_mask(pl_context *c) {
  if (!c->coarse.enabled || !(c->dist.active || c->coarseL.enabled)) return PL_OK;
  hipLaunchKernelGGL(k_local_mask, dim3(grid_for(c->N)), dim3(pl::kBlock), 0, c->stream, c->N, c->fixedbits.p,
                     c->sharedbits.p, c->maskL.p);
  PL_HIP(hipGetLastError());
  return PL_OK;
}

inline int tile_modes_now(const pl_context *c) {
  return (c->coarse.tile_level && c->coarse.tile_modes == 12 && !c->coarseL.enabled) ? 12 : 6;
}

int launch_tile_blocks(pl_context *c, hipStream_t st) {
  pl::Coarse &cs = c->coarse;
  if (!cs.enabled || !c->have_bc || !cs.tile_level) return PL_OK;
  if (cs.cm == 12) return PL_OK;
  const uint8_t *fb = c->dist.active ? c->maskL.p : c->fixedbits.p;
  const bool twelve = tile_modes_now(c) == 12;
  if (!twelve)
    hipLaunchKernelGGL(pl::k_tile_blocks, dim3((unsigned)cs.n_tiles), dim3(pl::kBlock), 0, st, c->tile.tile_start.p,
                       c->tile.home_ptr.p, c->tile.foreign_ptr.p, c->tile.foreign_idx.p,
                       reinterpret_cast<const int2 *>(c->conn.p), c->rec.p, cs.agg_of_tile.p, cs.cen.p, c->xyz.p,
                       fb, cs.Bt_inv, (double *)nullptr);
  if (twelve) {
    hipLaunchKernelGGL(pl::k_tile_blocks_strain<true>, dim3((unsigned)cs.n_tiles), dim3(pl::kBlock), 0, st,
                       c->tile.tile_start.p, c->tile.home_ptr.p, c->tile.foreign_ptr.p, c->tile.foreign_idx.p,
                       reinterpret_cast<const int2 *>(c->conn.p), c->rec.p, cs.agg_of_tile.p, cs.cen.p, c->xyz.p, fb,
                       cs.Bt_raw);
    hipLaunchKernelGGL(pl::k_tile_blocks_strain<false>, dim3((unsigned)cs.n_tiles), dim3(pl::kBlock), 0, st,
                       c->tile.tile_start.p, c->tile.home_ptr.p, c->tile.foreign_ptr.p, c->tile.foreign_idx.p,
                       reinterpret_cast<const int2 *>(c->conn.p), c->rec.p, cs.agg_of_tile.p, cs.cen.p, c->xyz.p, fb,
                       cs.Bt_raw);
    hipLaunchKernelGGL(pl::k_tile_invert12, dim3((unsigned)cs.n_tiles), dim3(pl::kInv12Block), 0, st, cs.n_tiles,
                       (const double *)cs.Bt_raw, cs.Bt_inv);
  }
  PL_HIP(hipGetLastError());
  return PL_OK;
}

int build_coarse_level(pl_context *c, pl::Coarse &cs, const uint8_t *mask, bool reduce,
                       const std::function<void(int)> &after_chol = nullptr) {
  cs.ready = false;
  if (!cs.enabled || !c->have_bc) {
    if (after_chol) after_chol(1);
    return PL_OK;
  }
  bool tile_invert_pending = false;
  const int n = cs.ncp;
  if (!cs.ac_clean) PL_HIP(hipMemsetAsync(cs.Ac, 0, (size_t)n * n * sizeof(double), c->stream));
  cs.ac_clean = false;
  PL_HIP(hipMemsetAsync(cs.info, 0, 2 * sizeof(int), c->stream));
  if (cs.cm == 12) {
    const dim3 gt((unsigned)cs.n_tiles), blk(pl::kBlock);
    const int2 *conn2 = reinterpret_cast<const int2 *>(c->conn.p);
    const bool two_sets = c->dist.active;
    if (two_sets) {
      if (!cs.Bt_rawA && hipMalloc((void **)&cs.Bt_rawA, (size_t)cs.n_tiles * 144 * sizeof(double)) != hipSuccess)
        return fail(PL_ERR_HIP, "pl_assemble: out of device memory for the tile blocks");
      hipLaunchKernelGGL(pl::k_tile_blocks_strain<true>, gt, blk, 0, c->stream, c->tile.tile_start.p, c->tile.home_ptr.p,
                         c->tile.foreign_ptr.p, c->tile.foreign_idx.p, conn2, c->rec.p, cs.agg_of_tile.p, cs.cen.p,
                         c->xyz.p, (const uint8_t *)c->maskL.p, cs.Bt_raw);
      hipLaunchKernelGGL(pl::k_tile_blocks_strain<false>, gt, blk, 0, c->stream, c->tile.tile_start.p, c->tile.home_ptr.p,
                         c->tile.foreign_ptr.p, c->tile.foreign_idx.p, conn2, c->rec.p, cs.agg_of_tile.p, cs.cen.p,
                         c->xyz.p, (const uint8_t *)c->maskL.p, cs.Bt_raw);
    }
    double *rawA = two_sets ? cs.Bt_rawA : cs.Bt_raw;
    PL_HIP(hipEventRecord(c->ev_t0, c->stream));
    PL_HIP(hipStreamWaitEvent(c->side2, c->ev_t0, 0));
    hipLaunchKernelGGL(pl::k_tile_blocks_strain<true>, gt, blk, 0, c->side2, c->tile.tile_start.p, c->tile.home_ptr.p,
                       c->tile.foreign_ptr.p, c->tile.foreign_idx.p, conn2, c->rec.p, cs.agg_of_tile.p, cs.cen.p, c->xyz.p,
                       mask, rawA);
    if (cs.n_cross > 0)
      hipLaunchKernelGGL(pl::k_coarse_cross12, dim3(grid_for(cs.n_cross)), blk, 0, c->side2, cs.n_cross,
                         cs.cross_idx.p, c->conn.p, c->rec.p, cs.agg_of_node.p, cs.cen.p, c->xyz.p, mask, n, cs.Ac);
    PL_HIP(hipEventRecord(c->ev_t1, c->side2));
    hipLaunchKernelGGL(pl::k_tile_blocks_strain<false>, gt, blk, 0, c->stream, c->tile.tile_start.p, c->tile.home_ptr.p,
                       c->tile.foreign_ptr.p, c->tile.foreign_idx.p, conn2, c->rec.p, cs.agg_of_tile.p, cs.cen.p, c->xyz.p,
                       mask, rawA);
    PL_HIP(hipStreamWaitEvent(c->stream, c->ev_t1, 0));
    hipLaunchKernelGGL(pl::k_agg_add_tiles, dim3(grid_for(cs.n_tiles * 144)), blk, 0, c->stream, cs.n_tiles,
                       cs.agg_of_tile.p, (const double *)rawA, n, cs.Ac);
    PL_HIP(hipEventRecord(c->ev_t0, c->stream));
    PL_HIP(hipStreamWaitEvent(c->side2, c->ev_t0, 0));
    hipLaunchKernelGGL(pl::k_tile_invert12, dim3((unsigned)cs.n_tiles), dim3(pl::kInv12Block), 0,
                       c->side2, cs.n_tiles, (const double *)cs.Bt_raw, cs.Bt_inv);
    PL_HIP(hipEventRecord(c->ev_t1, c->side2));
    tile_invert_pending = true;
  } else {
  if (cs.n_fix < 0) {
    if (!cs.fix_count) PL_HIP(hipMalloc((void **)&cs.fix_count, sizeof(int)));
    int cnt = 0;
    DevBuf<int64_t> keys;
    for (int pass = 0; pass < 2; ++pass) {
      PL_HIP(hipMemsetAsync(cs.fix_count, 0, sizeof(int), c->stream));
      hipLaunchKernelGGL(pl::k_list_fixed_struts, dim3(grid_for(c->B)), dim3(pl::kBlock), 0, c->stream, c->B,
                         c->conn.p, cs.agg_of_node.p, mask, pass ? keys.p : (int64_t *)nullptr, cs.fix_count);
      if (pass == 0) {
        PL_HIP(hipMemcpyAsync(&cnt, cs.fix_count, sizeof(int), hipMemcpyDeviceToHost, c->stream));
        PL_HIP(hipStreamSynchronize(c->stream));
        if (cnt == 0) break;
        PL_HIP(keys.alloc((size_t)cnt));
      }
    }
    std::vector<int32_t> list;
    if (cnt > 0) {
      std::vector<int64_t> hk((size_t)cnt);
      PL_HIP(hipMemcpyAsync(hk.data(), keys.p, hk.size() * sizeof(int64_t), hipMemcpyDeviceToHost, c->stream));
      PL_HIP(hipStreamSynchronize(c->stream));
      std::sort(hk.begin(), hk.end());
      list.reserve(hk.size() + hk.size() / 4 + pl::kWave);
      for (size_t q = 0; q < hk.size(); ++q) {
        if (q > 0 && (hk[q] >> 32) != (hk[q - 1] >> 32))
          while (list.size() % pl::kWave) list.push_back(-1);
        list.push_back((int32_t)(hk[q] & 0xffffffffLL));
      }
      while (list.size() % pl::kWave) list.push_back(-1);
      PL_HIP(cs.fix_list.upload(list));
    }
    cs.n_fix = (int64_t)list.size();
  }
  if (cs.n_fix > 0)
    hipLaunchKernelGGL(pl::k_coarse_assemble, dim3(grid_for(cs.n_fix)), dim3(pl::kBlock), 0, c->stream, cs.n_fix,
                       cs.fix_list.p, c->conn.p, c->rec.p, cs.agg_of_node.p, cs.cen.p, c->xyz.p, mask, n,
                       cs.Ac);
  if (cs.n_cross > 0)
    hipLaunchKernelGGL(pl::k_coarse_assemble_cross, dim3(grid_for(cs.n_cross)), dim3(pl::kBlock), 0, c->stream,
                       cs.n_cross, cs.cross_idx.p, c->conn.p, c->rec.p, cs.agg_of_node.p, cs.cen.p, c->xyz.p,
                       mask, n, cs.Ac);
  }
  if (reduce && c->dist.active) {
    const int nb = n / pl::kNB;
    if (cs.bw_blocks > 0 && cs.bw_blocks + 1 < nb) {
      const int64_t cnt = (int64_t)n * (cs.bw_blocks + 1) * pl::kNB;
      hipLaunchKernelGGL(pl::k_band_pack, dim3((unsigned)((cnt + 255) / 256)), dim3(256), 0, c->stream, n, n,
                         cs.bw_blocks, cs.Ac, cs.Lf);
      if (pl::dist_sum_scalars(c->dist, cs.Lf, (int)cnt, c->stream))
        return fail(PL_ERR_HIP, "RCCL all-reduce of the coarse operator failed");
      hipLaunchKernelGGL(pl::k_band_unpack, dim3((unsigned)((cnt + 255) / 256)), dim3(256), 0, c->stream, n, n,
                         cs.bw_blocks, cs.Lf, cs.Ac);
    } else if (pl::dist_sum_scalars(c->dist, cs.Ac, n * n, c->stream)) {
      return fail(PL_ERR_HIP, "RCCL all-reduce of the coarse operator failed");
    }
  }
  hipLaunchKernelGGL(pl::k_coarse_regularize, dim3((n + 255) / 256), dim3(256), 0, c->stream, n, cs.Ac);
  pl::TrtriPhases ph;
  {
    const char *e = std::getenv("PL_TRTRI_ROWS");
    ph.rows = e ? std::atoi(e) : 3;
    ph.stream = c->side2;
    ph.ev_go = c->ev_p0;
    ph.ev_done = c->ev_p1;
  }
  pl::coarse_factor(cs, n, c->stream, after_chol, c->opt.chol_persistent ? cs.bar : (unsigned *)nullptr, ph);
  cs.ainv_ready = false;
  if (&cs == &c->coarse && (small_wanted(c) || (n <= pl::kOneGemvMaxDofs && c->opkind == 0))) {
    if (!cs.Ainv && hipMalloc((void **)&cs.Ainv, (size_t)n * n * sizeof(float)) != hipSuccess)
      return fail(PL_ERR_HIP, "pl_assemble: out of device memory for the explicit inverse of the dense level");
    const long tiles = (long)(n / 32) * (n / 32 + 1) / 2;
    if (cs.w16)
      hipLaunchKernelGGL(pl::k_dense_explicit_inverse<pl::bf16_t>, dim3((unsigned)((tiles + 3) / 4)), dim3(256), 0, c->stream, n,
                         reinterpret_cast<const pl::bf16_t *>(cs.W), n, cs.Ainv);
    else
      hipLaunchKernelGGL(pl::k_dense_explicit_inverse<float>, dim3((unsigned)((tiles + 3) / 4)), dim3(256), 0, c->stream, n,
                         (const float *)cs.W, n, cs.Ainv);
    cs.ainv_ready = true;
  }
  if (tile_invert_pending) PL_HIP(hipStreamWaitEvent(c->stream, c->ev_t1, 0));
  PL_HIP(hipGetLastError());
  int info[2] = {0, 0};
  PL_HIP(hipMemcpyAsync(info, cs.info, sizeof(info), hipMemcpyDeviceToHost, c->stream));
  PL_HIP(hipStreamSynchronize(c->stream));
  if (&cs == &c->coarse) c->coarse_info = info[0];
  cs.ready = (info[0] == 0);
  return PL_OK;
}

int build_coarse(pl_context *c, const std::function<void(int)> &after_chol = nullptr) {
  int rc = build_coarse_level(c, c->coarse, c->fixedbits.p, true, after_chol);
  if (rc || !c->coarseL.enabled) return rc;
  return build_coarse_level(c, c->coarseL, c->maskL.p, false);
}

inline const double *cinv(const pl_context *c) { return c->cls_ready ? c->cls_table.p : c->kcc_inv.p; }
inline const uint16_t *ccls(const pl_context *c) { return c->cls_ready ? c->cls_id.p : (const uint16_t *)nullptr; }

int select_condensed(pl_context *c, const std::vector<uint8_t> &bits) {
  c->cond_ready = false;
  c->n_cond = 0;
  c->cond_agree = -1;
  const bool wanted = c->opt.condense >= 0 && c->opkind == 0 && c->coarse.enabled && c->opt.precision != 2 &&
                      !c->h_cand.empty();
  if (!wanted) return PL_OK;
  const int64_t N = c->N;
  std::vector<int32_t> picked;
  for (int64_t i = 0; i < N; ++i)
    if (c->h_cand[i] && !bits[i] && (c->h_shared.empty() || !c->h_shared[i])) picked.push_back((int32_t)i);
  if (picked.empty()) return PL_OK;
  std::vector<uint8_t> flag((size_t)N, 0), mask(bits);
  for (int32_t i : picked) {
    flag[i] = 1;
    mask[i] = 0x3f;
  }
  PL_HIP(c->cnodes.alloc(picked.size()));
  PL_HIP(c->kcc_inv.alloc(picked.size() * 36));
  if (!c->maskC.p) {
    PL_HIP(c->maskC.alloc(N));
    PL_HIP(c->cflag.alloc(N));
  }
  PL_HIP(hipMemcpy(c->cnodes.p, picked.data(), picked.size() * sizeof(int32_t), hipMemcpyHostToDevice));
  {
    std::vector<int32_t> keep;
    keep.reserve((size_t)N - picked.size());
    for (int64_t i = 0; i < N; ++i)
      if (!flag[i]) keep.push_back((int32_t)i);
    PL_HIP(c->ckeep.alloc(std::max<size_t>(1, keep.size())));
    if (!keep.empty()) PL_HIP(hipMemcpy(c->ckeep.p, keep.data(), keep.size() * sizeof(int32_t), hipMemcpyHostToDevice));
  }
  if (!c->cbase.p) PL_HIP(c->cbase.alloc(N));
  c->cbase_state = -1;
  PL_HIP(hipMemcpy(c->maskC.p, mask.data(), N, hipMemcpyHostToDevice));
  PL_HIP(hipMemcpy(c->cflag.p, flag.data(), N, hipMemcpyHostToDevice));
  if (!c->cend.p) PL_HIP(c->cend.alloc(c->B));
  hipLaunchKernelGGL(k_cond_ends, dim3(grid_for(c->B)), dim3(pl::kBlock), 0, c->stream, c->B,
                     reinterpret_cast<const int2 *>(c->conn.p), (const uint8_t *)c->cflag.p, c->cend.p);
  refresh_visit_words(c, c->stream);
  if (refresh_visit_words_dir(c, c->stream)) return PL_ERR_HIP;
  PL_HIP(hipGetLastError());
  c->n_cond = (int64_t)picked.size();
  return PL_OK;
}
int agree_condensed(pl_context *c) {
  if (!c->dist.active || c->cond_agree != -1) return PL_OK;
  const bool asked = c->opt.condense >= 0 && c->opkind == 0 && c->coarse.enabled && c->opt.precision != 2;
  if (!asked) {
// ... 172 lines not shown
```

pylatticedso_amd/csrc/pl_coarse.h:

```cpp
#pragma once
#include <hip/hip_runtime.h>

#include <algorithm>
#include <cstdint>
#include <vector>

#include "pl_dense.h"
#include "pl_kernels.h"
#include "pl_tile.h"

namespace pl {


struct Coarse {
  bool enabled = false;
  bool ready = false;
  int n_agg = 0, nc = 0, ncp = 0;
  int cm = 6;
  int bw_blocks = 0;
  int64_t n_tiles = 0;
  int vblock = kBlock;
  TBuf<int32_t> agg_of_node, agg_of_tile;
  TBuf<int32_t> tile_of_node;
  TBuf<double> cen;
// ... 448 lines not shown
#pragma unroll
    for (int k = 0; k < 6; ++k)
      if (k < j) s -= L[j * 6 + k] * L[j * 6 + k];
    keep[j] = s > 1e-12 * dmax;
    if (!keep[j]) {
#pragma unroll
      for (int k = 0; k < 6; ++k) L[j * 6 + k] = 0.0;
      L[j * 6 + j] = 1.0;
      continue;
    }
    const double d = sqrt(s);
    L[j * 6 + j] = d;
#pragma unroll
    for (int i = 0; i < 6; ++i)
      if (i > j) {
        double v = 0.5 * (A[i * 6 + j] + A[j * 6 + i]);
#pragma unroll
        for (int k = 0; k < 6; ++k)
          if (k < j) v -= L[i * 6 + k] * L[j * 6 + k];
        L[i * 6 + j] = v / d;
      }
  }
  double W[36];
#pragma unroll
  for (int e = 0; e < 36; ++e) W[e] = 0.0;
#pragma unroll
  for (int j = 0; j < 6; ++j) {
    W[j * 6 + j] = 1.0 / L[j * 6 + j];
#pragma unroll
    for (int i = 0; i < 6; ++i)
      if (i > j) {
        double v = 0.0;
#pragma unroll
        for (int k = 0; k < 6; ++k)
          if (k >= j && k < i) v -= L[i * 6 + k] * W[k * 6 + j];
        W[i * 6 + j] = v / L[i * 6 + i];
      }
  }
#pragma unroll
  for (int i = 0; i < 6; ++i)
#pragma unroll
    for (int j = 0; j < 6; ++j) {
      double v = 0.0;
#pragma unroll
      for (int k = 0; k < 6; ++k)
        if (k >= i && k >= j) v += W[k * 6 + i] * W[k * 6 + j];
      A[i * 6 + j] = (keep[i] && keep[j]) ? v : 0.0;
    }
}

__global__ void k_band_pack(int n, int ld, int bwb, double *__restrict__ A, double *__restrict__ P) {
  const int W = (bwb + 1) * kNB;
  const int64_t e = (int64_t)blockIdx.x * blockDim.x + threadIdx.x;
  if (e >= (int64_t)n * W) return;
  const int i = (int)(e / W), j = (i / kNB - bwb) * kNB + (int)(e % W);
  double v = 0.0;
  if (j >= 0) {
    v = A[(size_t)i * ld + j];
    A[(size_t)i * ld + j] = 0.0;
  }
  P[e] = v;
}
__global__ void k_band_unpack(int n, int ld, int bwb, const double *__restrict__ P, double *__restrict__ A) {
  const int W = (bwb + 1) * kNB;
  const int64_t e = (int64_t)blockIdx.x * blockDim.x + threadIdx.x;
  if (e >= (int64_t)n * W) return;
  const int i = (int)(e / W), j = (i / kNB - bwb) * kNB + (int)(e % W);
  if (j >= 0) A[(size_t)i * ld + j] = P[e];
}

__global__ __launch_bounds__(kBlock) void k_tile_blocks(const int32_t *__restrict__ tile_start,
                                                        const int64_t *__restrict__ home_ptr,
                                                        const int64_t *__restrict__ foreign_ptr,
                                                        const int32_t *__restrict__ foreign_idx,
                                                        const int2 *__restrict__ conn2, const Record *__restrict__ rec,
                                                        const int32_t *__restrict__ agg_of_tile,
                                                        const double *__restrict__ cen, const double *__restrict__ xyz,
                                                        const uint8_t *__restrict__ fixedbits,
                                                        double *__restrict__ Bt_inv,
                                                        double *__restrict__ raw ) {
  __shared__ double red[36][kBlock / kWave];
  __shared__ double A[36];
  const int t = blockIdx.x;
  const int n0 = tile_start[t], n1 = tile_start[t + 1];
  const int a = agg_of_tile[t];
  const double c0 = cen[3 * a], c1 = cen[3 * a + 1], c2 = cen[3 * a + 2];
  double acc[36];
#pragma unroll
  for (int e = 0; e < 36; ++e) acc[e] = 0.0;
  const int64_t h0 = home_ptr[t], h1 = home_ptr[t + 1], f0 = foreign_ptr[t], f1 = foreign_ptr[t + 1];
  const int64_t total = (h1 - h0) + (f1 - f0);
  for (int64_t q = threadIdx.x; q < total; q += kBlock) {
    const int64_t b = q < (h1 - h0) ? h0 + q : (int64_t)foreign_idx[f0 + (q - (h1 - h0))];
    const int2 cn = conn2[b];
    const bool ina = cn.x >= n0 && cn.x < n1, inb = cn.y >= n0 && cn.y < n1;
    const unsigned fa = fixedbits ? fixedbits[cn.x] : 0u, fb = fixedbits ? fixedbits[cn.y] : 0u;
    if (ina && inb && fa == 0u && fb == 0u) continue;
    const Record r = load_record(rec, b);
    const double rela[3] = {xyz[3 * (int64_t)cn.x] - c0, xyz[3 * (int64_t)cn.x + 1] - c1, xyz[3 * (int64_t)cn.x + 2] - c2};
    const double relb[3] = {xyz[3 * (int64_t)cn.y] - c0, xyz[3 * (int64_t)cn.y + 1] - c1, xyz[3 * (int64_t)cn.y + 2] - c2};
    double Kss[36], Kso[36], C[36];
    if (inb) {
      tip_blocks(r, Kss, Kso);
      coarse_block(Kss, fb, fb, relb, relb, C);
#pragma unroll
      for (int e = 0; e < 36; ++e) acc[e] += C[e];
      if (ina) {
        coarse_block(Kso, fb, fa, relb, rela, C);
#pragma unroll
        for (int e = 0; e < 36; ++e) acc[e] += C[e];
      }
    }
    if (ina) {
      tip_blocks(reversed(r), Kss, Kso);
      coarse_block(Kss, fa, fa, rela, rela, C);
#pragma unroll
      for (int e = 0; e < 36; ++e) acc[e] += C[e];
      if (inb) {
        coarse_block(Kso, fa, fb, rela, relb, C);
#pragma unroll
        for (int e = 0; e < 36; ++e) acc[e] += C[e];
      }
    }
  }
  const int lane = threadIdx.x & 63, wv = threadIdx.x >> 6;
#pragma unroll
  for (int e = 0; e < 36; ++e) {
    const double s = wave_sum(acc[e]);
    if (lane == 0) red[e][wv] = s;
  }
  __syncthreads();
  if (threadIdx.x < 36) {
    double s = 0.0;
#pragma unroll
    for (int q = 0; q < kBlock / kWave; ++q) s += red[threadIdx.x][q];
    A[threadIdx.x] = s;
  }
  __syncthreads();
  if (raw) {
    if (threadIdx.x < 36) raw[(size_t)t * 144 + (threadIdx.x / 6) * 12 + threadIdx.x % 6] = A[threadIdx.x];
    return;
  }
  if (threadIdx.x == 0) {
    double M[36];
#pragma unroll
    for (int e = 0; e < 36; ++e) M[e] = A[e];
    spd6_inverse(M);
#pragma unroll
    for (int e = 0; e < 36; ++e) Bt_inv[(size_t)t * 36 + e] = M[e];
  }
}

template <bool RIGID>
__global__ __launch_bounds__(kBlock) void k_tile_blocks_strain(const int32_t *__restrict__ tile_start,
                                                               const int64_t *__restrict__ home_ptr,
                                                               const int64_t *__restrict__ foreign_ptr,
                                                               const int32_t *__restrict__ foreign_idx,
                                                               const int2 *__restrict__ conn2,
                                                               const Record *__restrict__ rec,
                                                               const int32_t *__restrict__ agg_of_tile,
                                                               const double *__restrict__ cen,
                                                               const double *__restrict__ xyz,
                                                               const uint8_t *__restrict__ fixedbits,
                                                               double *__restrict__ raw) {
  __shared__ double red[57][kBlock / kWave];
  const int t = blockIdx.x;
  const int n0 = tile_start[t], n1 = tile_start[t + 1];
  const int a = agg_of_tile[t];
  const double c0 = cen[3 * a], c1 = cen[3 * a + 1], c2 = cen[3 * a + 2];
  double SS[21], RS[RIGID ? 1 : 36];
  double RR[RIGID ? 21 : 1];
#pragma unroll
  for (int e = 0; e < (RIGID ? 21 : 1); ++e) RR[e] = 0.0;
#pragma unroll
  for (int e = 0; e < 21; ++e) SS[e] = 0.0;
#pragma unroll
  for (int e = 0; e < (RIGID ? 1 : 36); ++e) RS[e] = 0.0;
  const int64_t h0 = home_ptr[t], h1 = home_ptr[t + 1], f0 = foreign_ptr[t], f1 = foreign_ptr[t + 1];
  const int64_t total = (h1 - h0) + (f1 - f0);
  for (int64_t v = threadIdx.x; v < total; v += kBlock) {
    const int64_t b = v < (h1 - h0) ? h0 + v : (int64_t)foreign_idx[f0 + (v - (h1 - h0))];
    const int2 cn = conn2[b];
    const bool ina = cn.x >= n0 && cn.x < n1, inb = cn.y >= n0 && cn.y < n1;
    if (!ina && !inb) continue;
    const unsigned fa = fixedbits ? fixedbits[cn.x] : 0u, fb = fixedbits ? fixedbits[cn.y] : 0u;
    const bool free_inside = ina && inb && fa == 0u && fb == 0u;
    if (RIGID && free_inside) continue;
    const Record r = load_record(rec, b);
    const double rela[3] = {xyz[3 * (int64_t)cn.x] - c0, xyz[3 * (int64_t)cn.x + 1] - c1, xyz[3 * (int64_t)cn.x + 2] - c2};
    const double relb[3] = {xyz[3 * (int64_t)cn.y] - c0, xyz[3 * (int64_t)cn.y + 1] - c1, xyz[3 * (int64_t)cn.y + 2] - c2};
    const V3 d = {r.dx, r.dy, r.dz}, zero = {0.0, 0.0, 0.0};
#pragma unroll
    for (int q = 0; q < (RIGID ? 0 : 6); ++q) {
      const V3 uA = ina ? mask3(strain_disp(q, rela), fa) : zero, uB = inb ? mask3(strain_disp(q, relb), fb) : zero;
      V3 F, M;
      tip_force(r, uA, zero, uB, zero, F, M);
      const V3 FB = mask3(F, fb), MB = mask3(M, fb >> 3);
      const V3 FA = mask3((-1.0) * F, fa), MA = mask3((-1.0) * M - cross(d, F), fa >> 3);
      double s6[6] = {0, 0, 0, 0, 0, 0};
      if (inb) strain_restrict(FB, relb, s6, 1.0);
      if (ina) strain_restrict(FA, rela, s6, 1.0);
#pragma unroll
      for (int p = 0; p <= q; ++p) SS[q * (q + 1) / 2 + p] += s6[p];
      if (!free_inside) {
        if (inb) {
          RS[0 * 6 + q] += FB.x;
          RS[1 * 6 + q] += FB.y;
          RS[2 * 6 + q] += FB.z;
          RS[3 * 6 + q] += MB.x + (relb[1] * FB.z - relb[2] * FB.y);
          RS[4 * 6 + q] += MB.y + (relb[2] * FB.x - relb[0] * FB.z);
          RS[5 * 6 + q] += MB.z + (relb[0] * FB.y - relb[1] * FB.x);
        }
        if (ina) {
          RS[0 * 6 + q] += FA.x;
          RS[1 * 6 + q] += FA.y;
          RS[2 * 6 + q] += FA.z;
          RS[3 * 6 + q] += MA.x + (rela[1] * FA.z - rela[2] * FA.y);
          RS[4 * 6 + q] += MA.y + (rela[2] * FA.x - rela[0] * FA.z);
          RS[5 * 6 + q] += MA.z + (rela[0] * FA.y - rela[1] * FA.x);
        }
      }
    }
    if (RIGID && !free_inside) {
#pragma unroll
      for (int q = 0; q < 6; ++q) {
        V3 uA = zero, tA = zero, uB = zero, tB = zero;
        if (ina) {
          mode_disp(q, rela, uA, tA);
          uA = mask3(uA, fa);
          tA = mask3(tA, fa >> 3);
        }
        if (inb) {
          mode_disp(q, relb, uB, tB);
          uB = mask3(uB, fb);
          tB = mask3(tB, fb >> 3);
        }
        V3 F, M;
        tip_force(r, uA, tA, uB, tB, F, M);
        double x6[6] = {0, 0, 0, 0, 0, 0};
        if (inb) {
          const V3 FB = mask3(F, fb), MB = mask3(M, fb >> 3);
          x6[0] += FB.x;
          x6[1] += FB.y;
          x6[2] += FB.z;
          x6[3] += MB.x + (relb[1] * FB.z - relb[2] * FB.y);
          x6[4] += MB.y + (relb[2] * FB.x - relb[0] * FB.z);
          x6[5] += MB.z + (relb[0] * FB.y - relb[1] * FB.x);
        }
        if (ina) {
          const V3 FA = mask3((-1.0) * F, fa), MA = mask3((-1.0) * M - cross(d, F), fa >> 3);
          x6[0] += FA.x;
          x6[1] += FA.y;
          x6[2] += FA.z;
          x6[3] += MA.x + (rela[1] * FA.z - rela[2] * FA.y);
          x6[4] += MA.y + (rela[2] * FA.x - rela[0] * FA.z);
          x6[5] += MA.z + (rela[0] * FA.y - rela[1] * FA.x);
        }
#pragma unroll
        for (int p = 0; p <= q; ++p) RR[q * (q + 1) / 2 + p] += x6[p];
      }
    }
  }
  const int lane = threadIdx.x & 63, wv = threadIdx.x >> 6;
  double *B = raw + (size_t)t * 144;
  if (RIGID) {
#pragma unroll
    for (int e = 0; e < 21; ++e) {
      const double s0 = wave_sum(RR[e]);
      if (lane == 0) red[e][wv] = s0;
    }
    __syncthreads();
    if (threadIdx.x < 21) {
      double v = 0.0;
#pragma unroll
      for (int q = 0; q < kBlock / kWave; ++q) v += red[threadIdx.x][q];
      int q = 0;
      while ((q + 1) * (q + 2) / 2 <= (int)threadIdx.x) ++q;
      const int p = (int)threadIdx.x - q * (q + 1) / 2;
      B[p * 12 + q] = v;
      B[q * 12 + p] = v;
    }
    return;
  }
#pragma unroll
  for (int e = 0; e < 21; ++e) {
    const double s1 = wave_sum(SS[e]);
    if (lane == 0) red[e][wv] = s1;
  }
#pragma unroll
  for (int e = 0; e < (RIGID ? 1 : 36); ++e) {
    const double s2 = wave_sum(RS[e]);
    if (lane == 0) red[21 + e][wv] = s2;
  }
  __syncthreads();
  if (threadIdx.x < 57) {
    double v = 0.0;
#pragma unroll
    for (int q = 0; q < kBlock / kWave; ++q) v += red[threadIdx.x][q];
    if (threadIdx.x < 21) {
      int q = 0;
      while ((q + 1) * (q + 2) / 2 <= (int)threadIdx.x) ++q;
      const int p = (int)threadIdx.x - q * (q + 1) / 2;
      B[(6 + p) * 12 + 6 + q] = v;
      B[(6 + q) * 12 + 6 + p] = v;
    } else {
      const int e = (int)threadIdx.x - 21, p = e / 6, q = e % 6;
      B[p * 12 + 6 + q] = v;
      B[(6 + q) * 12 + p] = v;
    }
  }
}
constexpr int kInv12Block = 192;
__global__ __launch_bounds__(kInv12Block) void k_tile_invert12(int64_t T, const double *__restrict__ raw,
                                                              double *__restrict__ Bt_inv) {
  constexpr int n = 12;
  __shared__ double A[n][n + 1];
  __shared__ double diag0[n];
  const int64_t t = blockIdx.x;
  if (t >= T) return;
  const int e = threadIdx.x, i = e / n, j = e - n * i;
  const bool act = e < n * n;
  if (act) A[i][j] = 0.5 * (raw[t * 144 + i * n + j] + raw[t * 144 + j * n + i]);
  __syncthreads();
  if (e < n) diag0[e] = A[e][e];
  __syncthreads();
  unsigned dropped = 0u;
  for (int k = 0; k < n; ++k) {
    const double d = A[k][k];
    if (!(d > 1e-10 * diag0[k]) || !(diag0[k] > 0.0)) {
      dropped |= 1u << k;
      continue;
    }
    const double inv = 1.0 / d;
    double v = 0.0;
    if (act) {
      const bool di = (dropped >> i) & 1u, dj = (dropped >> j) & 1u;
      if (i == k && j == k) v = -inv;
      else if (i == k) v = A[k][j] * inv;
      else if (j == k) v = A[k][i] * inv;
      else if (di || dj) v = A[i][j];
      else v = A[i][j] - (A[i][k] * inv) * A[k][j];
    }
    __syncthreads();
    if (act) A[i][j] = v;
    __syncthreads();
  }
  if (act) {
    const bool out = ((dropped >> i) & 1u) || ((dropped >> j) & 1u);
    Bt_inv[t * 144 + i * n + j] = out ? 0.0 : -A[i][j];
  }
}
inline void coarse_factor(Coarse &cs, int n, hipStream_t s, const std::function<void(int)> &after_chol, unsigned *bar,
                          TrtriPhases ph = TrtriPhases()) {
  if (cs.w16)
    dense_factor_inverse(cs.Ac, cs.Lf, reinterpret_cast<bf16_t *>(cs.W), reinterpret_cast<bf16_t *>(cs.Wt), cs.Dinv, n, n,
                         cs.info, cs.bw_blocks, s, after_chol, bar, ph);
  else
    dense_factor_inverse(cs.Ac, cs.Lf, cs.W, cs.Wt, cs.Dinv, n, n, cs.info, cs.bw_blocks, s, after_chol, bar, ph);
}
constexpr int kOneGemvMaxDofs = 2048;
inline void coarse_apply(const Coarse &cs, const double *r, double *t, double *y, double *dot_out, const double *add0,
                         hipStream_t s) {
  static const bool one_off = [] { const char *e = std::getenv("PL_ONE_GEMV"); return e && e[0] == '0'; }();
  if (cs.ainv_ready && cs.Ainv && cs.ncp <= kOneGemvMaxDofs && !one_off) {
    hipLaunchKernelGGL(k_full_gemv, dim3((cs.ncp + 3) / 4), dim3(kBlock), 0, s, cs.ncp, (const float *)cs.Ainv, cs.ncp, r, y,
                       dot_out, add0);
    return;
  }
  if (cs.w16)
    dense_apply(reinterpret_cast<const bf16_t *>(cs.W), reinterpret_cast<const bf16_t *>(cs.Wt), cs.ncp, cs.ncp, r, t, y,
                dot_out, add0, s);
  else
    dense_apply(cs.W, cs.Wt, cs.ncp, cs.ncp, r, t, y, dot_out, add0, s);
}

__global__ __launch_bounds__(kBlock) void k_to_float(int64_t n, const double *__restrict__ x, float *__restrict__ y) {
  const int64_t i = (int64_t)blockIdx.x * kBlock + threadIdx.x;
  if (i < n) y[i] = (float)x[i];
}

template <typename PT, typename RT, int TM = 6, bool MULTI = true, bool LOCAL = true>
__global__ __launch_bounds__(kBlock) void k_pcg_update_tile(const int32_t *__restrict__ tile_start,
                                                            const int32_t *__restrict__ agg_of_tile,
                                                            const double *__restrict__ cen,
                                                            const double *__restrict__ xyz,
                                                            const PT *__restrict__ Ap,
                                                            const float *__restrict__ dinv32,
                                                            const double *__restrict__ w ,
                                                            RT *__restrict__ r,
                                                            double *__restrict__ scal, double *__restrict__ rc,
                                                            const double *__restrict__ Bt_inv ,
                                                            double *__restrict__ yt,
                                                            const int32_t *__restrict__ aggL_of_tile ,
                                                            const double *__restrict__ cenL,
                                                            const uint8_t *__restrict__ shared ,
                                                            double *__restrict__ rcL, int ncp,
                                                            const uint8_t *__restrict__ skip_rows ,
                                                            int cm = 6 ,
                                                            const float *__restrict__ rel32 = nullptr ) {
  __shared__ double red[32][4 * kBlock / kWave];
  if constexpr (!MULTI) {
    w = nullptr;
    shared = nullptr;
  }
  if constexpr (!MULTI || !LOCAL) aggL_of_tile = nullptr;
  double *rr_slot = rc + ncp + (blockIdx.x & (kSlots - 1)), *rdr_slot = rr_slot + kSlots;
  const int t = blockIdx.x;
  double pap, old_rz;
  scalar_read2(scal, S_PAP, S_RZ_OLD, pap, old_rz);
  const double alpha = (pap != 0.0) ? old_rz / pap : 0.0;
  const int n0 = tile_start[t], n1 = tile_start[t + 1];
  const int a = agg_of_tile[t];
  const double c0 = cen[3 * a], c1 = cen[3 * a + 1], c2 = cen[3 * a + 2];
  __shared__ double sbi[16][TM];
  double bi[TM];
#pragma unroll
  for (int j = 0; j < TM; ++j) bi[j] = 0.0;
  const int my_mode = (TM == 12) ? ((int)threadIdx.x < 6 ? (int)threadIdx.x : ((int)threadIdx.x >= 8 && (int)threadIdx.x < 14
                                                                                   ? (int)threadIdx.x - 2 : -1))
                                 : ((int)threadIdx.x < 6 ? (int)threadIdx.x : -1);
  if (Bt_inv && my_mode >= 0) {
#pragma unroll
    for (int j = 0; j < TM; ++j) bi[j] = Bt_inv[(size_t)t * (TM * TM) + TM * my_mode + j];
  }
  if (threadIdx.x < 16) {
#pragma unroll
    for (int j = 0; j < TM; ++j) sbi[threadIdx.x][j] = bi[j];
  }
  double accS[6] = {0, 0, 0, 0, 0, 0};
  double accD[6] = {0, 0, 0, 0, 0, 0};
  double acc[8] = {0, 0, 0, 0, 0, 0, 0, 0};
  const int aL = aggL_of_tile ? aggL_of_tile[t] : 0;
  double l0 = 0.0, l1 = 0.0, l2 = 0.0;
  if (aggL_of_tile) {
    l0 = cenL[3 * aL];
    l1 = cenL[3 * aL + 1];
    l2 = cenL[3 * aL + 2];
  }
  double accL[6] = {0, 0, 0, 0, 0, 0};
  double accT[6] = {0, 0, 0, 0, 0, 0};
  const bool own_t = Bt_inv && shared;
  for (int i = n0 + threadIdx.x; i < n1; i += blockDim.x) {
    if (skip_rows && skip_rows[i]) continue;
    double av[6], dv[6], rv[6];
    const float2 *d2 = reinterpret_cast<const float2 *>(dinv32 + 6 * (int64_t)i);
#pragma unroll
    for (int k = 0; k < 3; ++k) {
      const double2 aa = load_pair(Ap, 3 * (int64_t)i + k), rr = load_pair(r, 3 * (int64_t)i + k);
      const float2 dd = d2[k];
      av[2 * k] = aa.x; av[2 * k + 1] = aa.y;
      dv[2 * k] = dd.x; dv[2 * k + 1] = dd.y;
      rv[2 * k] = rr.x; rv[2 * k + 1] = rr.y;
    }
#pragma unroll
    for (int k = 0; k < 6; ++k) rv[k] -= alpha * av[k];
#pragma unroll
    for (int k = 0; k < 3; ++k) store_pair(r, 3 * (int64_t)i + k, double2{rv[2 * k], rv[2 * k + 1]});
    if (sizeof(RT) == 4) {
#pragma unroll
      for (int k = 0; k < 6; ++k) rv[k] = (double)(float)rv[k];
    }
    double wt[6] = {1, 1, 1, 1, 1, 1};
    if (w) {
// ... 569 lines not shown
```

pylatticedso_amd/csrc/pl_context.h:

```cpp
#pragma once
#include <hip/hip_runtime.h>

#include <algorithm>
#include <atomic>
#include <chrono>
#include <cmath>
#include <cstdlib>
#include <cstdio>
#include <cstring>
#include <functional>
#include <memory>
#include <numeric>
#include <string>
#include <vector>

#include "../../include/pylattice_hip.h"
#include "pl_kernels.h"
#include "pl_parallel.h"
#include "pl_tile.h"
#include "pl_rows.h"
#include "pl_dist.h"
#include "pl_coarse.h"
#include "pl_cg1.h"
#include "pl_small.h"
#include "pl_persist.h"
#include "pl_palette.h"
#include "pl_ddm.h"
#include "pl_lzone.h"

namespace {

thread_local std::string g_err;

int fail(int code, const std::string &msg) {
  g_err = msg;
  return code;
}

#define PL_HIP(expr)                                                                                   \
  do {                                                                                                 \
    hipError_t _e = (expr);                                                                            \
    if (_e != hipSuccess)                                                                              \
      return fail(PL_ERR_HIP, std::string(#expr) + ": " + hipGetErrorString(_e));                     \
  } while (0)

template <typename T>
struct DevBuf {
  T *p = nullptr;
  size_t n = 0;
  ~DevBuf() { release(); }
  void release() {
    if (p) (void)hipFree(p);
    p = nullptr;
    n = 0;
  }
  hipError_t alloc(size_t count) {
    release();
    n = count;
    if (count == 0) return hipSuccess;
    return hipMalloc(reinterpret_cast<void **>(&p), count * sizeof(T));
  }
};

inline unsigned grid_for(int64_t n, int block = pl::kBlock) { return (unsigned)((n + block - 1) / block); }
inline unsigned grid_stream(int64_t n) {
  return (unsigned)std::max<int64_t>(1, std::min<int64_t>((n + pl::kBlock - 1) / pl::kBlock, 2048));
}

}

struct pl_context {
  pl_opts_t opt{};
  pl::Material mat{};
  int64_t N = 0, B = 0;
  hipStream_t stream = nullptr;
  hipEvent_t ev0 = nullptr, ev1 = nullptr;
  hipStream_t side = nullptr;
  hipEvent_t ev_fork = nullptr, ev_join = nullptr, ev_chol = nullptr, ev_t0 = nullptr, ev_t1 = nullptr;
  hipEvent_t ev_p0 = nullptr, ev_p1 = nullptr;
  hipEvent_t ev_fill1 = nullptr;
  hipStream_t side2 = nullptr;
  hipStream_t side_cu = nullptr;
  bool assembled = false, have_bc = false, have_bsr = false;
  int pal_fallback_flags[2] = {1, 0};
  int *pal_host_flags = pal_fallback_flags;
  bool want_bsr = false;
  int bsr_with_bc = 0;

  std::vector<int32_t> perm, iperm;
  bool reordered = false;
  std::vector<int32_t> bperm;

  DevBuf<double> xyz, radius, seg_len;
  DevBuf<double> mult;
  DevBuf<int32_t> conn, seg_nsub;
  DevBuf<pl::Record> rec;
  DevBuf<double> rec5;
  DevBuf<int64_t> slice_ptr;
  DevBuf<int2> ent;
  int64_t n_slices = 0, n_ent = 0;
  int lpn = pl::kDefaultLPN;
  DevBuf<int64_t> bsr_rowptr;
  DevBuf<int32_t> bsr_col, ent_slot, diag_slot;
  DevBuf<double> bsr_vals;
  int64_t nblk = 0;
  std::vector<int64_t> h_rowptr;
  std::vector<int32_t> h_col;
  DevBuf<uint8_t> fixed;
  DevBuf<uint8_t> fixedbits;
  std::vector<uint8_t> h_fixedbits;
  DevBuf<double> ubar, f;
  DevBuf<double> diag, dinv, x, r, z, p, Ap, tmp, tmp2, scal, hist;
  DevBuf<double> xprev;
  bool xprev_valid = false;
  int pal_fail_streak = 0, pal_skip_left = 0;
  bool pal_skipped = false;
  DevBuf<double> xprev2;
  bool xprev2_valid = false;
  DevBuf<double> xprev3;
  bool xprev3_valid = false;
  static constexpr int kWarmMax = 8;
  DevBuf<double> gh[kWarmMax - 1];
  int gh_head = 0, gh_count = 0;
  DevBuf<double> gw[kWarmMax];
  DevBuf<double> gw_dots;
  DevBuf<double> cg1;
  int hist_cap = 0;
  pl::TilePlan tile;
  int opkind = 0;
  int64_t ddm_cells = 0;
  int ddm_nb = 0;
  int ddm_n_S = 0;
  std::vector<int32_t> h_ddm_cell_nodes, h_ddm_cell_S;
  DevBuf<int32_t> ddm_cell_nodes, ddm_cell_S;
  DevBuf<double> ddm_St;
  DevBuf<double> ddm_Sraw;
  DevBuf<int64_t> ddm_node_ptr;
  DevBuf<int32_t> ddm_node_ent;
  DevBuf<double> ddm_stage;
  DevBuf<int32_t> ddm_order;
  DevBuf<int32_t> ddm_tiles, ddm_tile_S;
  int64_t ddm_n_tiles = 0;
  DevBuf<int32_t> ddm_tile_gidx;
  DevBuf<int32_t> ddm_cell_P;
  DevBuf<double> ddm_Pt;
  bool ddm_have_P = false;
  DevBuf<double> dd_A, dd_Lf, dd_W, dd_Wt, dd_Dinv, dd_tv;
  DevBuf<int> dd_info;
  int dd_n = 0;
  int dd_bw = 0;
  bool dd_ready = false;
  DevBuf<double> dd_B;
  bool dd_blocks = false;
  DevBuf<double> dd2_xyz, dd2_cen;
  DevBuf<int32_t> dd2_agg, dd2_ptr, dd2_nodes;
  pl::Coarse dd2;
  int dd2_n_agg = 0;
  bool dd2_plan = false, dd2_ready = false;
  DevBuf<int> stop_flag;
  bool stop_use = false;
  double stop_thresh = 0.0;
  DevBuf<unsigned long long> pal_keys;
  DevBuf<int> pal_owner, pal_flags;
  DevBuf<uint16_t> pal_id;
  DevBuf<int> pal_dense_of_slot;
  DevBuf<pl::Record> pal_dense;
  DevBuf<uint32_t> vword;
  DevBuf<uint32_t> vword_dir;
  bool vword_dir_fresh = false;
  bool pal_lds = false;
  pl::RowPlan rows;
  DevBuf<uint32_t> rword;
  DevBuf<pl::Record> pal_dense2;
  bool pal_rows = false;
  DevBuf<pl::Record> palette;
  bool pal_ready = false;
  int pal_entries = 0;
  pl::Coarse coarse;
  int coarse_info = 0;
  pl::Coarse coarseL;
  DevBuf<uint8_t> sharedbits, maskL;
  std::vector<uint8_t> h_cand;
  std::vector<uint8_t> h_shared;
  DevBuf<uint8_t> cend;
  DevBuf<int32_t> cnodes, cbase;
  DevBuf<int32_t> ckeep;
  int cbase_state = -1;
  DevBuf<double> kcc_inv;
  DevBuf<uint8_t> maskC, cflag;
  DevBuf<unsigned long long> cls_key, cls_keys;
  DevBuf<int> cls_owner, cls_flags;
  DevBuf<uint16_t> cls_id;
  DevBuf<double> cls_table;
  int *cls_host_flag = nullptr;
  bool cls_ready = false;
  DevBuf<double> p2, small_scal, small_rc;
  bool small_use = false;
  bool persist_use = false;
  DevBuf<double> ps_Ug, ps_red;
  DevBuf<unsigned> ps_flags;
  DevBuf<unsigned long long> ps_dbg;
  DevBuf<int32_t> ps_agg_ptr, ps_agg_idx;
  int ps_n_agg = 0;
  int last_iterations = 0;
  int64_t n_cond = 0;
  bool cond_ready = false;
  bool cond_use = false;
  int cond_agree = -1;
  pl::Dist dist;
  std::vector<int32_t> h_tile_start;
  DevBuf<int32_t> ov_iface, ov_inner;
  int64_t n_ov_iface = 0, n_ov_inner = 0;
  bool ov_ready = false;
  hipStream_t comm_stream = nullptr;
  hipEvent_t ev_ov_a = nullptr, ev_ov_x = nullptr;

  pl_stats_t last{};
  double ms_assembly = 0.0;
  double *pin6 = nullptr;
  size_t pin6_n = 0;
  DevBuf<int32_t> per_ptr, per_nodes;
  int64_t n_per_groups = 0;
  double *pinB = nullptr;
  DevBuf<double> sens_out;
  DevBuf<double> usol;
  bool usol_valid = false;
  std::shared_ptr<void> multi_ws;

  ~pl_context() {
    if (ev0) (void)hipEventDestroy(ev0);
    if (ev1) (void)hipEventDestroy(ev1);
    if (ev_fork) (void)hipEventDestroy(ev_fork);
    if (ev_join) (void)hipEventDestroy(ev_join);
    if (ev_chol) (void)hipEventDestroy(ev_chol);
    if (ev_fill1) (void)hipEventDestroy(ev_fill1);
    if (ev_p0) (void)hipEventDestroy(ev_p0);
    if (ev_p1) (void)hipEventDestroy(ev_p1);
    if (ev_t0) (void)hipEventDestroy(ev_t0);
    if (ev_t1) (void)hipEventDestroy(ev_t1);
    if (pin6) (void)hipHostFree(pin6);
    if (pinB) (void)hipHostFree(pinB);
    if (ev_ov_a) (void)hipEventDestroy(ev_ov_a);
    if (ev_ov_x) (void)hipEventDestroy(ev_ov_x);
    if (comm_stream) (void)hipStreamDestroy(comm_stream);
    if (side2) (void)hipStreamDestroy(side2);
    if (side_cu) (void)hipStreamDestroy(side_cu);
    if (side) (void)hipStreamDestroy(side);
    if (stream) (void)hipStreamDestroy(stream);
  }
};

namespace {

int staging(pl_context *c, double **out) {
  const size_t n6 = (size_t)c->N * 6;
  if (!c->pin6 || c->pin6_n < n6) {
    if (c->pin6) (void)hipHostFree(c->pin6);
    c->pin6 = nullptr;
    void *p = nullptr;
    PL_HIP(hipHostMalloc(&p, n6 * sizeof(double), hipHostMallocDefault));
    c->pin6 = static_cast<double *>(p);
    c->pin6_n = n6;
  }
  *out = c->pin6;
  return PL_OK;
}

int stagingB(pl_context *c, double **out) {
  if (!c->pinB) {
    void *p = nullptr;
    PL_HIP(hipHostMalloc(&p, (size_t)std::max<int64_t>(c->B, 1) * sizeof(double), hipHostMallocDefault));
    c->pinB = static_cast<double *>(p);
  }
  *out = c->pinB;
  return PL_OK;
}

int upload6(pl_context *c, const double *host, double *dev, std::vector<double> &) {
  const size_t n6 = (size_t)c->N * 6;
  double *st = nullptr;
  int rc = staging(c, &st);
  if (rc) return rc;
  if (!c->reordered) {
    pl::parallel_for((int64_t)n6, [&](int64_t b, int64_t e, unsigned) { std::memcpy(st + b, host + b, (e - b) * sizeof(double)); },
                     1 << 18);
  } else {
    pl::parallel_for(c->N, [&](int64_t b, int64_t e, unsigned) {
      for (int64_t i = b; i < e; ++i) std::memcpy(st + 6 * i, host + 6 * (size_t)c->perm[i], 6 * sizeof(double));
    }, 1 << 15);
  }
  PL_HIP(hipMemcpyAsync(dev, st, n6 * sizeof(double), hipMemcpyHostToDevice, c->stream));
  PL_HIP(hipStreamSynchronize(c->stream));
  return PL_OK;
}

int download6(pl_context *c, const double *dev, double *host) {
  const size_t n6 = (size_t)c->N * 6;
  double *st = nullptr;
  int rc = staging(c, &st);
  if (rc) return rc;
  PL_HIP(hipMemcpyAsync(st, dev, n6 * sizeof(double), hipMemcpyDeviceToHost, c->stream));
  PL_HIP(hipStreamSynchronize(c->stream));
  if (!c->reordered) {
    pl::parallel_for((int64_t)n6, [&](int64_t b, int64_t e, unsigned) { std::memcpy(host + b, st + b, (e - b) * sizeof(double)); },
                     1 << 18);
  } else {
    pl::parallel_for(c->N, [&](int64_t b, int64_t e, unsigned) {
      for (int64_t i = b; i < e; ++i) std::memcpy(host + 6 * (size_t)c->perm[i], st + 6 * i, 6 * sizeof(double));
    }, 1 << 15);
  }
  return PL_OK;
}

}
```

Baseline: 245.2 million.

## Use palette histogram table for free interior struts in 12-mode coarse tile blocks

Precomputes per-tile lists that split struts into free-interior and other struts. Free-interior struts are reduced through an LDS histogram of dense palette ids multiplied by a small precomputed SS table, so strain-mode tip forces are not recomputed for each of them. The cross-aggregate kernel moves to a third stream so it overlaps the tile kernels. In exchange, the tile lists are built once on the host with several blocking device-to-host copies, and a new event now orders the main stream after palette verification.

```diff
diff --git a/pylatticedso_amd/csrc/pl_api.hip b/pylatticedso_amd/csrc/pl_api.hip
--- a/pylatticedso_amd/csrc/pl_api.hip
+++ b/pylatticedso_amd/csrc/pl_api.hip
@@ -194,7 +194,10 @@
   PL_HIPC(hipEventCreateWithFlags(&c->ev_p0, hipEventDisableTiming));
   PL_HIPC(hipEventCreateWithFlags(&c->ev_p1, hipEventDisableTiming));
   PL_HIPC(hipEventCreateWithFlags(&c->ev_fill1, hipEventDisableTiming));
+  PL_HIPC(hipEventCreateWithFlags(&c->ev_pal, hipEventDisableTiming));
+  PL_HIPC(hipEventCreateWithFlags(&c->ev_t2, hipEventDisableTiming));
   PL_HIPC(hipStreamCreateWithFlags(&c->side2, hipStreamNonBlocking));
+  PL_HIPC(hipStreamCreateWithFlags(&c->side3, hipStreamNonBlocking));
   {
     const char *e = std::getenv("PL_BSR_CUMASK");
     const int k = e ? std::atoi(e) : 4;
@@ -901,6 +904,7 @@
   h->have_bc = true;
   h->coarse.n_fix = -1;
   h->coarseL.n_fix = -1;
+  h->tl_ready = false;
   {
     int rcs = select_condensed(h, bits);
     if (rcs) return rcs;
@@ -1138,6 +1142,8 @@
   }
   int rc = agree_condensed(h);
   if (rc) return rc;
+  rc = build_tile_lists(h);
+  if (rc) return rc;
   PL_HIP(hipEventRecord(h->ev0, h->stream));
   rc = launch_records(h);
   if (rc) return rc;
@@ -1209,6 +1215,7 @@
   PL_HIP(hipEventRecord(h->ev1, h->stream));
   PL_HIP(hipStreamSynchronize(h->stream));
   finish_palette(h);
+  h->pal_attempt_now = false;
   finish_condensed_classes(h);
   for (pl::Coarse *cs : {&h->coarse, &h->coarseL})
     if (cs->ready && cs->Ac) {
@@ -1967,6 +1974,13 @@
         }
         return r11 ? r11 : pcg_tail_coarse_t<float, float>(h, cur, nxt, k, p32, (const float *)Ap32, x32, r32);
       }
+      case 12: {
+        pl::Coarse &cs = h->coarse;
+        if (!(cs.enabled && cs.cm == 12 && h->have_bc && !h->dist.active))
+          return fail(PL_ERR_STATE, "pl_time_kernel: 12 needs the 12-mode dense level of a single-GPU handle");
+        const char *e = std::getenv("PL_TILE_HIST");
+        return launch_front12(h, cs, h->fixedbits.p, cs.Bt_raw, h->tl_front_hist && h->tl_ready && !(e && e[0] == '0'));
+      }
       default: return fail(PL_ERR_ARG, "pl_time_kernel: unknown kernel id");
     }
   };
@@ -1980,6 +1994,8 @@
     if (rc) return rc;
   }
   PL_HIP(hipEventRecord(h->ev1, h->stream));
+  if (which == 12)
+    PL_HIP(hipMemsetAsync(h->coarse.Ac, 0, (size_t)h->coarse.ncp * h->coarse.ncp * sizeof(double), h->stream));
   PL_HIP(hipStreamSynchronize(h->stream));
   float ms = 0.f;
   PL_HIP(hipEventElapsedTime(&ms, h->ev0, h->ev1));
diff --git a/pylatticedso_amd/csrc/pl_assembly.h b/pylatticedso_amd/csrc/pl_assembly.h
--- a/pylatticedso_amd/csrc/pl_assembly.h
+++ b/pylatticedso_amd/csrc/pl_assembly.h
@@ -42,6 +42,7 @@
 }
 
 int launch_palette(pl_context *c, hipStream_t st) {
+  c->pal_attempt_now = false;
   c->pal_ready = false;
   c->pal_lds = false;
   c->pal_rows = false;
@@ -87,6 +88,8 @@
   hipLaunchKernelGGL(pl::k_pal_publish, g, blk, 0, st, c->B, c->rec.p, c->pal_owner.p, c->pal_id.p, c->palette.p);
   hipLaunchKernelGGL(pl::k_pal_verify, g, blk, 0, st, c->B, c->rec.p, c->pal_id.p, c->palette.p, c->pal_owner.p,
                      c->pal_flags.p, c->pal_dense_of_slot.p, c->pal_dense.p, pl::kPalDenseMax);
+  PL_HIP(hipEventRecord(c->ev_pal, st));
+  c->pal_attempt_now = true;
   refresh_visit_words(c, st);
   if (c->pal_dense2.p)
     hipLaunchKernelGGL(pl::k_pal_orient, dim3(1), dim3(pl::kPalDenseMax), 0, st, pl::kPalDenseMax, c->pal_dense.p,
@@ -201,6 +204,123 @@
   return PL_OK;
 }
 
+int build_tile_lists(pl_context *c) {
+  const pl::Coarse &cs = c->coarse;
+  static_assert(pl::kTileHistIds == pl::kPalDenseMax, "the LDS histogram holds every dense palette id");
+  if (c->tl_ready || !cs.enabled || cs.cm != 12 || !c->have_bc || c->dist.active || !c->opt.palette || !c->tile.ready ||
+      c->opkind != 0)
+    return PL_OK;
+  const int64_t T = cs.n_tiles, B = c->B;
+  std::vector<int32_t> ts((size_t)T + 1), conn((size_t)2 * B), fidx((size_t)std::max<int64_t>(1, c->tile.n_foreign));
+  std::vector<int64_t> hp((size_t)T + 1), fp((size_t)T + 1);
+  PL_HIP(hipMemcpy(ts.data(), c->tile.tile_start.p, ts.size() * sizeof(int32_t), hipMemcpyDeviceToHost));
+  PL_HIP(hipMemcpy(hp.data(), c->tile.home_ptr.p, hp.size() * sizeof(int64_t), hipMemcpyDeviceToHost));
+  PL_HIP(hipMemcpy(fp.data(), c->tile.foreign_ptr.p, fp.size() * sizeof(int64_t), hipMemcpyDeviceToHost));
+  if (c->tile.n_foreign > 0)
+    PL_HIP(hipMemcpy(fidx.data(), c->tile.foreign_idx.p, (size_t)c->tile.n_foreign * sizeof(int32_t), hipMemcpyDeviceToHost));
+  PL_HIP(hipMemcpy(conn.data(), c->conn.p, conn.size() * sizeof(int32_t), hipMemcpyDeviceToHost));
+  const std::vector<uint8_t> &bits = c->h_fixedbits;
+  auto strut_of = [&](int64_t t, int64_t v) { return v < hp[t + 1] - hp[t] ? hp[t] + v : (int64_t)fidx[fp[t] + (v - (hp[t + 1] - hp[t]))]; };
+  auto kind_of = [&](int64_t t, int64_t b) {
+    const int32_t a = conn[2 * b], d = conn[2 * b + 1];
+    const bool ina = a >= ts[t] && a < ts[t + 1], inb = d >= ts[t] && d < ts[t + 1];
+    if (!ina && !inb) return 0;
+    return (ina && inb && bits[a] == 0 && bits[d] == 0) ? 1 : 2;
+  };
+  std::vector<int64_t> free_ptr((size_t)T + 1, 0), other_ptr((size_t)T + 1, 0);
+  pl::parallel_for(T, [&](int64_t t0, int64_t t1, unsigned) {
+    for (int64_t t = t0; t < t1; ++t) {
+      const int64_t total = (hp[t + 1] - hp[t]) + (fp[t + 1] - fp[t]);
+      int64_t nf = 0, no = 0;
+      for (int64_t v = 0; v < total; ++v) {
+        const int k = kind_of(t, strut_of(t, v));
+        nf += k == 1;
+        no += k == 2;
+      }
+      free_ptr[t + 1] = nf;
+      other_ptr[t + 1] = no;
+    }
+  }, 64);
+  for (int64_t t = 0; t < T; ++t) {
+    free_ptr[t + 1] += free_ptr[t];
+    other_ptr[t + 1] += other_ptr[t];
+  }
+  std::vector<int32_t> free_idx((size_t)std::max<int64_t>(1, free_ptr[T])), other_idx((size_t)std::max<int64_t>(1, other_ptr[T]));
+  pl::parallel_for(T, [&](int64_t t0, int64_t t1, unsigned) {
+    for (int64_t t = t0; t < t1; ++t) {
+      const int64_t total = (hp[t + 1] - hp[t]) + (fp[t + 1] - fp[t]);
+      int64_t qf = free_ptr[t], qo = other_ptr[t];
+      for (int64_t v = 0; v < total; ++v) {
+        const int64_t b = strut_of(t, v);
+        const int k = kind_of(t, b);
+        if (k == 1) free_idx[qf++] = (int32_t)b;
+        else if (k == 2) other_idx[qo++] = (int32_t)b;
+      }
+    }
+  }, 64);
+  PL_HIP(c->tl_free_ptr.alloc(free_ptr.size()));
+  PL_HIP(c->tl_other_ptr.alloc(other_ptr.size()));
+  PL_HIP(c->tl_free_idx.alloc(free_idx.size()));
+  PL_HIP(c->tl_other_idx.alloc(other_idx.size()));
+  if (!c->tl_table.p) PL_HIP(c->tl_table.alloc((size_t)pl::kTileHistIds * 21));
+  PL_HIP(hipMemcpy(c->tl_free_ptr.p, free_ptr.data(), free_ptr.size() * sizeof(int64_t), hipMemcpyHostToDevice));
+  PL_HIP(hipMemcpy(c->tl_other_ptr.p, other_ptr.data(), other_ptr.size() * sizeof(int64_t), hipMemcpyHostToDevice));
+  PL_HIP(hipMemcpy(c->tl_free_idx.p, free_idx.data(), free_idx.size() * sizeof(int32_t), hipMemcpyHostToDevice));
+  PL_HIP(hipMemcpy(c->tl_other_idx.p, other_idx.data(), other_idx.size() * sizeof(int32_t), hipMemcpyHostToDevice));
+  c->tl_ready = true;
+  return PL_OK;
+}
+
+int launch_front12(pl_context *c, pl::Coarse &cs, const uint8_t *mask, double *rawA, bool lists) {
+  const int n = cs.ncp;
+  const dim3 gt((unsigned)cs.n_tiles), blk(pl::kBlock);
+  const int2 *conn2 = reinterpret_cast<const int2 *>(c->conn.p);
+  PL_HIP(hipEventRecord(c->ev_t0, c->stream));
+  PL_HIP(hipStreamWaitEvent(c->side2, c->ev_t0, 0));
+  if (lists) {
+    if (cs.n_cross > 0) {
+      PL_HIP(hipStreamWaitEvent(c->side3, c->ev_t0, 0));
+      hipLaunchKernelGGL(pl::k_coarse_cross12, dim3(grid_for(cs.n_cross)), blk, 0, c->side3, cs.n_cross, cs.cross_idx.p,
+                         c->conn.p, c->rec.p, cs.agg_of_node.p, cs.cen.p, c->xyz.p, mask, n, cs.Ac);
+      PL_HIP(hipEventRecord(c->ev_t2, c->side3));
+    }
+    hipLaunchKernelGGL(pl::k_tile_blocks_strain_list<true>, gt, blk, 0, c->side2, c->tile.tile_start.p, c->tl_free_ptr.p,
+                       c->tl_free_idx.p, c->tl_other_ptr.p, c->tl_other_idx.p, conn2, c->rec.p, cs.agg_of_tile.p, cs.cen.p,
+                       c->xyz.p, mask, (const int *)c->pal_flags.p, (const uint16_t *)c->pal_id.p,
+                       (const int *)c->pal_dense_of_slot.p, (const double *)c->tl_table.p, rawA);
+    PL_HIP(hipEventRecord(c->ev_t1, c->side2));
+    PL_HIP(hipStreamWaitEvent(c->stream, c->ev_pal, 0));
+    hipLaunchKernelGGL(pl::k_tile_ss_table, dim3(1), dim3(pl::kTileHistIds), 0, c->stream, (const int *)c->pal_flags.p,
+                       (const pl::Record *)c->pal_dense.p, c->tl_table.p);
+    hipLaunchKernelGGL(pl::k_tile_blocks_strain_list<false>, gt, blk, 0, c->stream, c->tile.tile_start.p, c->tl_free_ptr.p,
+                       c->tl_free_idx.p, c->tl_other_ptr.p, c->tl_other_idx.p, conn2, c->rec.p, cs.agg_of_tile.p, cs.cen.p,
+                       c->xyz.p, mask, (const int *)c->pal_flags.p, (const uint16_t *)c->pal_id.p,
+                       (const int *)c->pal_dense_of_slot.p, (const double *)c->tl_table.p, rawA);
+    if (cs.n_cross > 0) PL_HIP(hipStreamWaitEvent(c->stream, c->ev_t2, 0));
+  } else {
+    hipLaunchKernelGGL(pl::k_tile_blocks_strain<true>, gt, blk, 0, c->side2, c->tile.tile_start.p, c->tile.home_ptr.p,
+                       c->tile.foreign_ptr.p, c->tile.foreign_idx.p, conn2, c->rec.p, cs.agg_of_tile.p, cs.cen.p, c->xyz.p,
+                       mask, rawA);
+    if (cs.n_cross > 0)
+      hipLaunchKernelGGL(pl::k_coarse_cross12, dim3(grid_for(cs.n_cross)), blk, 0, c->side2, cs.n_cross,
+                         cs.cross_idx.p, c->conn.p, c->rec.p, cs.agg_of_node.p, cs.cen.p, c->xyz.p, mask, n, cs.Ac);
+    PL_HIP(hipEventRecord(c->ev_t1, c->side2));
+    hipLaunchKernelGGL(pl::k_tile_blocks_strain<false>, gt, blk, 0, c->stream, c->tile.tile_start.p, c->tile.home_ptr.p,
+                       c->tile.foreign_ptr.p, c->tile.foreign_idx.p, conn2, c->rec.p, cs.agg_of_tile.p, cs.cen.p, c->xyz.p,
+                       mask, rawA);
+  }
+  PL_HIP(hipStreamWaitEvent(c->stream, c->ev_t1, 0));
+  hipLaunchKernelGGL(pl::k_agg_add_tiles, dim3(grid_for(cs.n_tiles * 144)), blk, 0, c->stream, cs.n_tiles,
+                     cs.agg_of_tile.p, (const double *)rawA, n, cs.Ac);
+  PL_HIP(hipGetLastError());
+  return PL_OK;
+}
+inline bool front_lists_now(const pl_context *c, const pl::Coarse &cs, const uint8_t *mask) {
+  const char *e = std::getenv("PL_TILE_HIST");
+  return !(e && e[0] == '0') && &cs == &c->coarse && cs.cm == 12 && !c->dist.active && mask == c->fixedbits.p &&
+         c->tl_ready && c->pal_attempt_now && c->pal_flags.p && c->pal_id.p && c->tl_table.p;
+}
+
 int build_coarse_level(pl_context *c, pl::Coarse &cs, const uint8_t *mask, bool reduce,
                        const std::function<void(int)> &after_chol = nullptr) {
   cs.ready = false;
@@ -228,21 +348,11 @@
                          c->xyz.p, (const uint8_t *)c->maskL.p, cs.Bt_raw);
     }
     double *rawA = two_sets ? cs.Bt_rawA : cs.Bt_raw;
-    PL_HIP(hipEventRecord(c->ev_t0, c->stream));
-    PL_HIP(hipStreamWaitEvent(c->side2, c->ev_t0, 0));
-    hipLaunchKernelGGL(pl::k_tile_blocks_strain<true>, gt, blk, 0, c->side2, c->tile.tile_start.p, c->tile.home_ptr.p,
-                       c->tile.foreign_ptr.p, c->tile.foreign_idx.p, conn2, c->rec.p, cs.agg_of_tile.p, cs.cen.p, c->xyz.p,
-                       mask, rawA);
-    if (cs.n_cross > 0)
-      hipLaunchKernelGGL(pl::k_coarse_cross12, dim3(grid_for(cs.n_cross)), blk, 0, c->side2, cs.n_cross,
-                         cs.cross_idx.p, c->conn.p, c->rec.p, cs.agg_of_node.p, cs.cen.p, c->xyz.p, mask, n, cs.Ac);
-    PL_HIP(hipEventRecord(c->ev_t1, c->side2));
-    hipLaunchKernelGGL(pl::k_tile_blocks_strain<false>, gt, blk, 0, c->stream, c->tile.tile_start.p, c->tile.home_ptr.p,
-                       c->tile.foreign_ptr.p, c->tile.foreign_idx.p, conn2, c->rec.p, cs.agg_of_tile.p, cs.cen.p, c->xyz.p,
-                       mask, rawA);
-    PL_HIP(hipStreamWaitEvent(c->stream, c->ev_t1, 0));
-    hipLaunchKernelGGL(pl::k_agg_add_tiles, dim3(grid_for(cs.n_tiles * 144)), blk, 0, c->stream, cs.n_tiles,
-                       cs.agg_of_tile.p, (const double *)rawA, n, cs.Ac);
+    if (&cs == &c->coarse) c->tl_front_hist = front_lists_now(c, cs, mask);
+    {
+      int rcf = launch_front12(c, cs, mask, rawA, &cs == &c->coarse && c->tl_front_hist);
+      if (rcf) return rcf;
+    }
     PL_HIP(hipEventRecord(c->ev_t0, c->stream));
     PL_HIP(hipStreamWaitEvent(c->side2, c->ev_t0, 0));
     hipLaunchKernelGGL(pl::k_tile_invert12, dim3((unsigned)cs.n_tiles), dim3(pl::kInv12Block), 0,
diff --git a/pylatticedso_amd/csrc/pl_coarse.h b/pylatticedso_amd/csrc/pl_coarse.h
--- a/pylatticedso_amd/csrc/pl_coarse.h
+++ b/pylatticedso_amd/csrc/pl_coarse.h
@@ -624,6 +624,134 @@
 }
 
 template <bool RIGID>
+__device__ __forceinline__ void tile_strut_sums(const Record &r, const double *rela, const double *relb, bool ina, bool inb,
+                                                unsigned fa, unsigned fb, double *SS, double *RS, double *RR) {
+  const bool free_inside = ina && inb && fa == 0u && fb == 0u;
+  const V3 d = {r.dx, r.dy, r.dz}, zero = {0.0, 0.0, 0.0};
+#pragma unroll
+  for (int q = 0; q < (RIGID ? 0 : 6); ++q) {
+    const V3 uA = ina ? mask3(strain_disp(q, rela), fa) : zero, uB = inb ? mask3(strain_disp(q, relb), fb) : zero;
+    V3 F, M;
+    tip_force(r, uA, zero, uB, zero, F, M);
+    const V3 FB = mask3(F, fb), MB = mask3(M, fb >> 3);
+    const V3 FA = mask3((-1.0) * F, fa), MA = mask3((-1.0) * M - cross(d, F), fa >> 3);
+    double s6[6] = {0, 0, 0, 0, 0, 0};
+    if (inb) strain_restrict(FB, relb, s6, 1.0);
+    if (ina) strain_restrict(FA, rela, s6, 1.0);
+#pragma unroll
+    for (int p = 0; p <= q; ++p) SS[q * (q + 1) / 2 + p] += s6[p];
+    if (!free_inside) {
+      if (inb) {
+        RS[0 * 6 + q] += FB.x;
+        RS[1 * 6 + q] += FB.y;
+        RS[2 * 6 + q] += FB.z;
+        RS[3 * 6 + q] += MB.x + (relb[1] * FB.z - relb[2] * FB.y);
+        RS[4 * 6 + q] += MB.y + (relb[2] * FB.x - relb[0] * FB.z);
+        RS[5 * 6 + q] += MB.z + (relb[0] * FB.y - relb[1] * FB.x);
+      }
+      if (ina) {
+        RS[0 * 6 + q] += FA.x;
+        RS[1 * 6 + q] += FA.y;
+        RS[2 * 6 + q] += FA.z;
+        RS[3 * 6 + q] += MA.x + (rela[1] * FA.z - rela[2] * FA.y);
+        RS[4 * 6 + q] += MA.y + (rela[2] * FA.x - rela[0] * FA.z);
+        RS[5 * 6 + q] += MA.z + (rela[0] * FA.y - rela[1] * FA.x);
+      }
+    }
+  }
+  if (RIGID && !free_inside) {
+#pragma unroll
+    for (int q = 0; q < 6; ++q) {
+      V3 uA = zero, tA = zero, uB = zero, tB = zero;
+      if (ina) {
+        mode_disp(q, rela, uA, tA);
+        uA = mask3(uA, fa);
+        tA = mask3(tA, fa >> 3);
+      }
+      if (inb) {
+        mode_disp(q, relb, uB, tB);
+        uB = mask3(uB, fb);
+        tB = mask3(tB, fb >> 3);
+      }
+      V3 F, M;
+      tip_force(r, uA, tA, uB, tB, F, M);
+      double x6[6] = {0, 0, 0, 0, 0, 0};
+      if (inb) {
+        const V3 FB = mask3(F, fb), MB = mask3(M, fb >> 3);
+        x6[0] += FB.x;
+        x6[1] += FB.y;
+        x6[2] += FB.z;
+        x6[3] += MB.x + (relb[1] * FB.z - relb[2] * FB.y);
+        x6[4] += MB.y + (relb[2] * FB.x - relb[0] * FB.z);
+        x6[5] += MB.z + (relb[0] * FB.y - relb[1] * FB.x);
+      }
+      if (ina) {
+        const V3 FA = mask3((-1.0) * F, fa), MA = mask3((-1.0) * M - cross(d, F), fa >> 3);
+        x6[0] += FA.x;
+        x6[1] += FA.y;
+        x6[2] += FA.z;
+        x6[3] += MA.x + (rela[1] * FA.z - rela[2] * FA.y);
+        x6[4] += MA.y + (rela[2] * FA.x - rela[0] * FA.z);
+        x6[5] += MA.z + (rela[0] * FA.y - rela[1] * FA.x);
+      }
+#pragma unroll
+      for (int p = 0; p <= q; ++p) RR[q * (q + 1) / 2 + p] += x6[p];
+    }
+  }
+}
+template <bool RIGID>
+__device__ __forceinline__ void tile_strut_store(double (*red)[kBlock / kWave], const double *SS, const double *RS,
+                                                 const double *RR, double *B, double extra) {
+  const int lane = threadIdx.x & 63, wv = threadIdx.x >> 6;
+  if (RIGID) {
+#pragma unroll
+    for (int e = 0; e < 21; ++e) {
+      const double s0 = wave_sum(RR[e]);
+      if (lane == 0) red[e][wv] = s0;
+    }
+    __syncthreads();
+    if (threadIdx.x < 21) {
+      double v = 0.0;
+#pragma unroll
+      for (int q = 0; q < kBlock / kWave; ++q) v += red[threadIdx.x][q];
+      int q = 0;
+      while ((q + 1) * (q + 2) / 2 <= (int)threadIdx.x) ++q;
+      const int p = (int)threadIdx.x - q * (q + 1) / 2;
+      B[p * 12 + q] = v;
+      B[q * 12 + p] = v;
+    }
+    return;
+  }
+#pragma unroll
+  for (int e = 0; e < 21; ++e) {
+    const double s1 = wave_sum(SS[e]);
+    if (lane == 0) red[e][wv] = s1;
+  }
+#pragma unroll
+  for (int e = 0; e < (RIGID ? 1 : 36); ++e) {
+    const double s2 = wave_sum(RS[e]);
+    if (lane == 0) red[21 + e][wv] = s2;
+  }
+  __syncthreads();
+  if (threadIdx.x < 57) {
+    double v = 0.0;
+#pragma unroll
+    for (int q = 0; q < kBlock / kWave; ++q) v += red[threadIdx.x][q];
+    if (threadIdx.x < 21) {
+      v += extra;
+      int q = 0;
+      while ((q + 1) * (q + 2) / 2 <= (int)threadIdx.x) ++q;
+      const int p = (int)threadIdx.x - q * (q + 1) / 2;
+      B[(6 + p) * 12 + 6 + q] = v;
+      B[(6 + q) * 12 + 6 + p] = v;
+    } else {
+      const int e = (int)threadIdx.x - 21, p = e / 6, q = e % 6;
+      B[p * 12 + 6 + q] = v;
+      B[(6 + q) * 12 + p] = v;
+    }
+  }
+}
+template <bool RIGID>
 __global__ __launch_bounds__(kBlock) void k_tile_blocks_strain(const int32_t *__restrict__ tile_start,
                                                                const int64_t *__restrict__ home_ptr,
                                                                const int64_t *__restrict__ foreign_ptr,
@@ -661,126 +789,108 @@
     const Record r = load_record(rec, b);
     const double rela[3] = {xyz[3 * (int64_t)cn.x] - c0, xyz[3 * (int64_t)cn.x + 1] - c1, xyz[3 * (int64_t)cn.x + 2] - c2};
     const double relb[3] = {xyz[3 * (int64_t)cn.y] - c0, xyz[3 * (int64_t)cn.y + 1] - c1, xyz[3 * (int64_t)cn.y + 2] - c2};
-    const V3 d = {r.dx, r.dy, r.dz}, zero = {0.0, 0.0, 0.0};
-#pragma unroll
-    for (int q = 0; q < (RIGID ? 0 : 6); ++q) {
-      const V3 uA = ina ? mask3(strain_disp(q, rela), fa) : zero, uB = inb ? mask3(strain_disp(q, relb), fb) : zero;
-      V3 F, M;
-      tip_force(r, uA, zero, uB, zero, F, M);
-      const V3 FB = mask3(F, fb), MB = mask3(M, fb >> 3);
-      const V3 FA = mask3((-1.0) * F, fa), MA = mask3((-1.0) * M - cross(d, F), fa >> 3);
-      double s6[6] = {0, 0, 0, 0, 0, 0};
-      if (inb) strain_restrict(FB, relb, s6, 1.0);
-      if (ina) strain_restrict(FA, rela, s6, 1.0);
-#pragma unroll
-      for (int p = 0; p <= q; ++p) SS[q * (q + 1) / 2 + p] += s6[p];
-      if (!free_inside) {
-        if (inb) {
-          RS[0 * 6 + q] += FB.x;
-          RS[1 * 6 + q] += FB.y;
-          RS[2 * 6 + q] += FB.z;
-          RS[3 * 6 + q] += MB.x + (relb[1] * FB.z - relb[2] * FB.y);
-          RS[4 * 6 + q] += MB.y + (relb[2] * FB.x - relb[0] * FB.z);
-          RS[5 * 6 + q] += MB.z + (relb[0] * FB.y - relb[1] * FB.x);
-        }
-        if (ina) {
-          RS[0 * 6 + q] += FA.x;
-          RS[1 * 6 + q] += FA.y;
-          RS[2 * 6 + q] += FA.z;
-          RS[3 * 6 + q] += MA.x + (rela[1] * FA.z - rela[2] * FA.y);
-          RS[4 * 6 + q] += MA.y + (rela[2] * FA.x - rela[0] * FA.z);
-          RS[5 * 6 + q] += MA.z + (rela[0] * FA.y - rela[1] * FA.x);
-        }
-      }
-    }
-    if (RIGID && !free_inside) {
-#pragma unroll
-      for (int q = 0; q < 6; ++q) {
-        V3 uA = zero, tA = zero, uB = zero, tB = zero;
-        if (ina) {
-          mode_disp(q, rela, uA, tA);
-          uA = mask3(uA, fa);
-          tA = mask3(tA, fa >> 3);
-        }
-        if (inb) {
-          mode_disp(q, relb, uB, tB);
-          uB = mask3(uB, fb);
-          tB = mask3(tB, fb >> 3);
-        }
-        V3 F, M;
-        tip_force(r, uA, tA, uB, tB, F, M);
-        double x6[6] = {0, 0, 0, 0, 0, 0};
-        if (inb) {
-          const V3 FB = mask3(F, fb), MB = mask3(M, fb >> 3);
-          x6[0] += FB.x;
-          x6[1] += FB.y;
-          x6[2] += FB.z;
-          x6[3] += MB.x + (relb[1] * FB.z - relb[2] * FB.y);
-          x6[4] += MB.y + (relb[2] * FB.x - relb[0] * FB.z);
-          x6[5] += MB.z + (relb[0] * FB.y - relb[1] * FB.x);
-        }
-        if (ina) {
-          const V3 FA = mask3((-1.0) * F, fa), MA = mask3((-1.0) * M - cross(d, F), fa >> 3);
-          x6[0] += FA.x;
-          x6[1] += FA.y;
-          x6[2] += FA.z;
-          x6[3] += MA.x + (rela[1] * FA.z - rela[2] * FA.y);
-          x6[4] += MA.y + (rela[2] * FA.x - rela[0] * FA.z);
-          x6[5] += MA.z + (rela[0] * FA.y - rela[1] * FA.x);
-        }
-#pragma unroll
-        for (int p = 0; p <= q; ++p) RR[q * (q + 1) / 2 + p] += x6[p];
-      }
-    }
-  }
+    tile_strut_sums<RIGID>(r, rela, relb, ina, inb, fa, fb, SS, RS, RR);
+  }
+  tile_strut_store<RIGID>(red, SS, RS, RR, raw + (size_t)t * 144, 0.0);
+}
+
+constexpr int kTileHistIds = 256;
+__device__ __forceinline__ bool tile_hist_ok(const int *__restrict__ pal_flags) {
+  return pal_flags[0] == 0 && pal_flags[1] > 0 && pal_flags[1] <= kTileHistIds;
+}
+__global__ __launch_bounds__(kTileHistIds) void k_tile_ss_table(const int *__restrict__ pal_flags,
+                                                                const Record *__restrict__ pal_dense,
+                                                                double *__restrict__ table ) {
+  if (!tile_hist_ok(pal_flags)) return;
+  const int id = threadIdx.x;
+  if (id >= pal_flags[1]) return;
+  const Record r = load_record(pal_dense, id);
+  const double rela[3] = {0.0, 0.0, 0.0}, relb[3] = {r.dx, r.dy, r.dz};
+  double SS[21], RS[36], RR[1] = {0.0};
+#pragma unroll
+  for (int e = 0; e < 21; ++e) SS[e] = 0.0;
+#pragma unroll
+  for (int e = 0; e < 36; ++e) RS[e] = 0.0;
+  tile_strut_sums<false>(r, rela, relb, true, true, 0u, 0u, SS, RS, RR);
+#pragma unroll
+  for (int e = 0; e < 21; ++e) table[id * 21 + e] = SS[e];
+}
+template <bool RIGID>
+__global__ __launch_bounds__(kBlock) void k_tile_blocks_strain_list(const int32_t *__restrict__ tile_start,
+                                                                    const int64_t *__restrict__ free_ptr,
+                                                                    const int32_t *__restrict__ free_idx,
+                                                                    const int64_t *__restrict__ other_ptr,
+                                                                    const int32_t *__restrict__ other_idx,
+                                                                    const int2 *__restrict__ conn2,
+                                                                    const Record *__restrict__ rec,
+                                                                    const int32_t *__restrict__ agg_of_tile,
+                                                                    const double *__restrict__ cen,
+                                                                    const double *__restrict__ xyz,
+                                                                    const uint8_t *__restrict__ fixedbits,
+                                                                    const int *__restrict__ pal_flags,
+                                                                    const uint16_t *__restrict__ pal_id,
+                                                                    const int *__restrict__ dense_of_slot,
+                                                                    const double *__restrict__ table,
+                                                                    double *__restrict__ raw) {
+  __shared__ double red[57][kBlock / kWave];
+  __shared__ int cnt[RIGID ? 1 : kBlock / kWave][RIGID ? 1 : kTileHistIds];
+  const int t = blockIdx.x;
+  const int n0 = tile_start[t], n1 = tile_start[t + 1];
+  const int a = agg_of_tile[t];
+  const double c0 = cen[3 * a], c1 = cen[3 * a + 1], c2 = cen[3 * a + 2];
+  double SS[21], RS[RIGID ? 1 : 36];
+  double RR[RIGID ? 21 : 1];
+#pragma unroll
+  for (int e = 0; e < (RIGID ? 21 : 1); ++e) RR[e] = 0.0;
+#pragma unroll
+  for (int e = 0; e < 21; ++e) SS[e] = 0.0;
+#pragma unroll
+  for (int e = 0; e < (RIGID ? 1 : 36); ++e) RS[e] = 0.0;
+  const int64_t o0 = other_ptr[t], n_other = other_ptr[t + 1] - o0, f0 = free_ptr[t], n_free = free_ptr[t + 1] - f0;
   const int lane = threadIdx.x & 63, wv = threadIdx.x >> 6;
-  double *B = raw + (size_t)t * 144;
-  if (RIGID) {
-#pragma unroll
-    for (int e = 0; e < 21; ++e) {
-      const double s0 = wave_sum(RR[e]);
-      if (lane == 0) red[e][wv] = s0;
-    }
+  const bool hist = !RIGID && tile_hist_ok(pal_flags);
+  if (hist) {
+#pragma unroll
+    for (int k = 0; k < kTileHistIds / kWave; ++k) cnt[RIGID ? 0 : wv][RIGID ? 0 : lane + kWave * k] = 0;
+    for (int64_t base = (int64_t)wv * kWave; base < n_free; base += kBlock) {
+      const bool valid = base + lane < n_free;
+      int id = 0;
+      if (valid) id = dense_of_slot[pal_id[free_idx[f0 + base + lane]]] & (kTileHistIds - 1);
+      unsigned long long todo = __ballot(valid);
+      while (todo) {
+        const int leader = __ffsll((long long)todo) - 1;
+        const int idl = __builtin_amdgcn_readlane(id, leader);
+        const unsigned long long same = __ballot(valid && id == idl) & todo;
+        if (lane == leader) cnt[RIGID ? 0 : wv][RIGID ? 0 : idl] += __popcll(same);
+        todo &= ~same;
+      }
+    }
+  }
+  const int64_t total = n_other + ((RIGID || hist) ? 0 : n_free);
+  for (int64_t v = threadIdx.x; v < total; v += kBlock) {
+    const int64_t b = v < n_other ? (int64_t)other_idx[o0 + v] : (int64_t)free_idx[f0 + (v - n_other)];
+    const int2 cn = conn2[b];
+    const bool ina = cn.x >= n0 && cn.x < n1, inb = cn.y >= n0 && cn.y < n1;
+    const unsigned fa = fixedbits ? fixedbits[cn.x] : 0u, fb = fixedbits ? fixedbits[cn.y] : 0u;
+    const Record r = load_record(rec, b);
+    const double rela[3] = {xyz[3 * (int64_t)cn.x] - c0, xyz[3 * (int64_t)cn.x + 1] - c1, xyz[3 * (int64_t)cn.x + 2] - c2};
+    const double relb[3] = {xyz[3 * (int64_t)cn.y] - c0, xyz[3 * (int64_t)cn.y + 1] - c1, xyz[3 * (int64_t)cn.y + 2] - c2};
+    tile_strut_sums<RIGID>(r, rela, relb, ina, inb, fa, fb, SS, RS, RR);
+  }
+  double extra = 0.0;
+  if (hist) {
     __syncthreads();
     if (threadIdx.x < 21) {
-      double v = 0.0;
-#pragma unroll
-      for (int q = 0; q < kBlock / kWave; ++q) v += red[threadIdx.x][q];
-      int q = 0;
-      while ((q + 1) * (q + 2) / 2 <= (int)threadIdx.x) ++q;
-      const int p = (int)threadIdx.x - q * (q + 1) / 2;
-      B[p * 12 + q] = v;
-      B[q * 12 + p] = v;
-    }
-    return;
-  }
-#pragma unroll
-  for (int e = 0; e < 21; ++e) {
-    const double s1 = wave_sum(SS[e]);
-    if (lane == 0) red[e][wv] = s1;
-  }
-#pragma unroll
-  for (int e = 0; e < (RIGID ? 1 : 36); ++e) {
-    const double s2 = wave_sum(RS[e]);
-    if (lane == 0) red[21 + e][wv] = s2;
-  }
-  __syncthreads();
-  if (threadIdx.x < 57) {
-    double v = 0.0;
-#pragma unroll
-    for (int q = 0; q < kBlock / kWave; ++q) v += red[threadIdx.x][q];
-    if (threadIdx.x < 21) {
-      int q = 0;
-      while ((q + 1) * (q + 2) / 2 <= (int)threadIdx.x) ++q;
-      const int p = (int)threadIdx.x - q * (q + 1) / 2;
-      B[(6 + p) * 12 + 6 + q] = v;
-      B[(6 + q) * 12 + 6 + p] = v;
-    } else {
-      const int e = (int)threadIdx.x - 21, p = e / 6, q = e % 6;
-      B[p * 12 + 6 + q] = v;
-      B[(6 + q) * 12 + p] = v;
-    }
-  }
+      const int n_ids = pal_flags[1];
+      for (int id = 0; id < n_ids; ++id) {
+        int c = 0;
+#pragma unroll
+        for (int w = 0; w < kBlock / kWave; ++w) c += cnt[RIGID ? 0 : w][RIGID ? 0 : id];
+        if (c) extra += (double)c * table[id * 21 + threadIdx.x];
+      }
+    }
+  }
+  tile_strut_store<RIGID>(red, SS, RS, RR, raw + (size_t)t * 144, extra);
 }
 constexpr int kInv12Block = 192;
 __global__ __launch_bounds__(kInv12Block) void k_tile_invert12(int64_t T, const double *__restrict__ raw,
diff --git a/pylatticedso_amd/csrc/pl_context.h b/pylatticedso_amd/csrc/pl_context.h
--- a/pylatticedso_amd/csrc/pl_context.h
+++ b/pylatticedso_amd/csrc/pl_context.h
@@ -80,6 +80,9 @@
   hipEvent_t ev_p0 = nullptr, ev_p1 = nullptr;
   hipEvent_t ev_fill1 = nullptr;
   hipStream_t side2 = nullptr;
+  hipStream_t side3 = nullptr;
+  hipEvent_t ev_pal = nullptr;
+  hipEvent_t ev_t2 = nullptr;
   hipStream_t side_cu = nullptr;
   bool assembled = false, have_bc = false, have_bsr = false;
   int pal_fallback_flags[2] = {1, 0};
@@ -176,6 +179,12 @@
   DevBuf<pl::Record> palette;
   bool pal_ready = false;
   int pal_entries = 0;
+  bool pal_attempt_now = false;
+  DevBuf<int64_t> tl_free_ptr, tl_other_ptr;
+  DevBuf<int32_t> tl_free_idx, tl_other_idx;
+  DevBuf<double> tl_table;
+  bool tl_ready = false;
+  bool tl_front_hist = false;
   pl::Coarse coarse;
   int coarse_info = 0;
   pl::Coarse coarseL;
@@ -238,11 +247,14 @@
     if (ev_p1) (void)hipEventDestroy(ev_p1);
     if (ev_t0) (void)hipEventDestroy(ev_t0);
     if (ev_t1) (void)hipEventDestroy(ev_t1);
+    if (ev_t2) (void)hipEventDestroy(ev_t2);
+    if (ev_pal) (void)hipEventDestroy(ev_pal);
     if (pin6) (void)hipHostFree(pin6);
     if (pinB) (void)hipHostFree(pinB);
     if (ev_ov_a) (void)hipEventDestroy(ev_ov_a);
     if (ev_ov_x) (void)hipEventDestroy(ev_ov_x);
     if (comm_stream) (void)hipStreamDestroy(comm_stream);
+    if (side3) (void)hipStreamDestroy(side3);
     if (side2) (void)hipStreamDestroy(side2);
     if (side_cu) (void)hipStreamDestroy(side_cu);
     if (side) (void)hipStreamDestroy(side);
```

After: 234.3 million. 4.5% lower.
